# tdavchev/DESIRE

Hardware: AMD Instinct MI355X
Metric: agent-trajectory-samples/sec (K=20, T_pred=40) (higher is better)
Workload: dtype f32; 1 GPU; BASELINE configs[1]: SDD-like synthetic windows, 32 agent slots/window, K=20, T_obs=8/T_pred=40, H=128, L=128, fp32, posterior CVAE, IOC 1 refinement, social grid 4x4, scene grid 64x64x32; 512 windows/step/GPU; windows_per_gpu=512, rows_per_gpu=327680, parallelism=scene-sharded x1

## Files before the change

### desire_amd/_build.py

```python
from __future__ import annotations

import hashlib
import os
import shutil
import subprocess
from concurrent.futures import ThreadPoolExecutor

HERE = os.path.dirname(os.path.abspath(__file__))
CSRC = os.path.join(HERE, "csrc")
LIB = os.path.join(HERE, "libdesire_hip.so")
SOURCES = ["api.hip", "api_pack.hip", "api_forward.hip", "api_peer.hip", "api_ops.hip", "kernels_gemm.hip", "kernels_conv.hip", "kernels_rnn.hip", "kernels_aux.hip", "kernels_rank.hip", "kernels_kde.hip", "kernels_select.hip", "kernels_joint.hip", "kernels_worlds.hip", "kernels_plan.hip", "kernels_modes.hip", "kernels_scene_modes.hip", "kernels_occ.hip", "kernels_recon.hip", "kernels_compact.hip", "kernels_bwd.hip", "kernels_bwd_x3.hip", "kernels_bwd_cl.hip", "kernels_bf16.hip", "kernels_bf16_cl.hip", "kernels_x3.hip", "kernels_x6.hip", "kernels_x6r2.hip", "kernels_scene.hip", "kernels_rng.hip", "kernels_rollout.hip", "train.hip", "backward.hip"]
FLAGS = ["--offload-arch=gfx950", "-O3", "-std=c++17", "-fPIC", "-Wno-unused-value", "-Wno-pass-failed"]
FLAGS += os.environ.get("DESIRE_HIPCC_FLAGS", "").split()
_SINK = ["-mllvm", "-sink-insts-to-avoid-spills"]
FILE_FLAGS = {f: list(_SINK) for f in ("kernels_bf16_cl.hip", "kernels_x3.hip")}
_extra = os.environ.get("DESIRE_FILE_FLAGS", "")
for _item in filter(None, _extra.split(";")):
    _f, _, _v = _item.partition("=")
    FILE_FLAGS[_f] = [x for x in _v.split(",") if x]


def _sha(paths, extra: str = "") -> str:
    h = hashlib.sha256(extra.encode())
    for p in paths:
        h.update(os.path.basename(p).encode())
        with open(p, "rb") as fh:
            h.update(fh.read())
    return h.hexdigest()


def _headers():
    return sorted(os.path.join(CSRC, f) for f in os.listdir(CSRC) if f.endswith(".h")) + [os.path.join(HERE, "..", "include", "desire_hip.h")]


def source_hash() -> str:
    srcs = sorted(os.path.join(CSRC, f) for f in os.listdir(CSRC) if f.endswith(".hip"))
    return _sha(srcs + _headers(), " ".join(FLAGS) + repr(sorted(FILE_FLAGS.items())))[:16]


def _read(path: str) -> str:
    try:
        with open(path) as fh:
            return fh.read().strip()
    except OSError:
        return ""


def build_lib(force: bool = False, verbose: bool = False) -> str:
    want = source_hash()
    objdir = os.path.join(HERE, "build")
    lib_stamp = os.path.join(objdir, "lib.stamp")
    if not force and os.path.exists(LIB) and _read(lib_stamp) == want:
        return LIB
    hipcc = shutil.which("hipcc") or "/opt/rocm/bin/hipcc"
    if not os.path.exists(hipcc):
        raise RuntimeError("hipcc not found: cannot build libdesire_hip.so")
    os.makedirs(objdir, exist_ok=True)
    hdrs = _headers()

    def cc(src: str) -> str:
        obj = os.path.join(objdir, src.replace(".hip", ".o"))
        flags = list(FLAGS) + FILE_FLAGS.get(src, [])
        if src == "api.hip":
            flags.append('-DDESIRE_SRC_HASH="%s"' % want)
        key = _sha([os.path.join(CSRC, src)] + hdrs, " ".join(flags))
        if not force and os.path.exists(obj) and _read(obj + ".stamp") == key:
            return obj
        cmd = [hipcc, *flags, "-c", os.path.join(CSRC, src), "-o", obj]
        r = subprocess.run(cmd, capture_output=True, text=True)
        if r.returncode != 0:
            raise RuntimeError("hipcc failed on %s:\n%s" % (src, r.stderr[-4000:]))
        if verbose and r.stderr:
            print(r.stderr)
        with open(obj + ".stamp", "w") as fh:
            fh.write(key)
        return obj

    with ThreadPoolExecutor(len(SOURCES)) as ex:
        objs = list(ex.map(cc, SOURCES))
    r = subprocess.run([hipcc, "--offload-arch=gfx950", "-shared", "-fPIC", "-o", LIB, *objs],
                       capture_output=True, text=True)
    if r.returncode != 0:
        raise RuntimeError("link failed:\n" + r.stderr[-4000:])
    with open(lib_stamp, "w") as fh:
        fh.write(want)
    return LIB


if __name__ == "__main__":
    print(build_lib(force=True, verbose=True))
```

### desire_amd/_lib.py

```python
from __future__ import annotations

import ctypes as C
import os
from typing import Dict, List, Tuple

import numpy as np

from .spec import Dims

LIB_PATH = os.environ.get("DESIRE_HIP_LIB") or os.path.join(os.path.dirname(os.path.abspath(__file__)), "libdesire_hip.so")

EXPORTS = [
    "desire_last_error", "desire_version", "desire_dims_size", "desire_build_hash", "desire_create", "desire_destroy", "desire_set_weight",
    "desire_finalize_weights", "desire_set_scene_grids", "desire_set_scene_images", "desire_encode", "desire_sample",
    "desire_ioc_refine", "desire_forward", "desire_read_buffer", "desire_neighbor_bins",
    "desire_scene_cells", "desire_set_profiling", "desire_get_profile", "desire_scene_cnn", "desire_losses",
    "desire_temporal_conv", "desire_feature_pooling", "desire_build_windows", "desire_gaussian_sample", "desire_ade_fde",
    "desire_set_training", "desire_backward", "desire_get_grad", "desire_grad_buffer",
    "desire_train_loss", "desire_adam_step", "desire_get_weight", "desire_clip_grads",
    "desire_device_buffer", "desire_ioc_step", "desire_ioc_finish", "desire_get_bin_table",
    "desire_graph_begin", "desire_graph_end", "desire_graph_launch", "desire_rollout", "desire_build_windows_la", "desire_adam_state",
    "desire_set_option", "desire_train_loss_async", "desire_set_head_loss",
    "desire_peer_export", "desire_peer_open", "desire_ioc_peer_pass", "desire_peer_close", "desire_peer_region", "desire_peer_open_ptr", "desire_peer_status",
    "desire_rank_samples", "desire_ranked_errors", "desire_kde_nll", "desire_select_diverse", "desire_joint_metrics",
    "desire_set_rng", "desire_set_rng_origin", "desire_rng_state", "desire_rng_fill", "desire_rollout_samples",
    "desire_set_recon_loss", "desire_recon_weights", "desire_occupancy", "desire_plan_risk", "desire_fit_modes",
    "desire_select_worlds", "desire_fit_scene_modes",
]
OCC_AT, OCC_UNTIL = 0, 1
OCC_MODES = {"at": OCC_AT, "until": OCC_UNTIL}
RNG_BITS, RNG_NORMAL, RNG_LATENT, RNG_ROLLOUT = 0, 1, 2, 3
DIST_FINAL, DIST_MEAN, DIST_MAX = 0, 1, 2
WORLD_ALL, WORLD_MEAN = 0, 1
RECON_MEAN, RECON_MIN, RECON_SOFTMIN = 0, 1, 2
RECON_MODES = {"mean": RECON_MEAN, "min": RECON_MIN, "softmin": RECON_SOFTMIN}
MODES_MAX, MODES_MAX_ITERS = 16, 32
KDE_LOG_FLOOR = -20.0


class DesireDims(C.Structure):
    _fields_ = [(n, C.c_int32) for n in
                ("n_scenes", "mno", "K", "T_obs", "T_pred", "H", "L", "S", "C", "Gh", "Gw", "n_grids",
                 "grid_size", "E_v", "iters", "posterior")] + \
               [(n, C.c_float) for n in ("nb_w", "nb_h", "sx", "sy")] + [(n, C.c_int32) for n in ("bin_mode", "bn_mode", "bf16", "ref_compat", "n_dec", "ioc_form", "ioc_split", "train_fp32_mask", "flags")]

    @classmethod
    def from_dims(cls, d: Dims) -> "DesireDims":
        return cls(d.n_scenes, d.mno, d.K, d.T_obs, d.T_pred, d.H, d.L, d.S, d.C, d.Gh, d.Gw, d.n_grids,
                   d.grid_size, d.E_v, d.iters, d.posterior, d.nb_w, d.nb_h, d.sx, d.sy, int(getattr(d, "bin_mode", 0)),
                   int(getattr(d, "bn_mode", 0)), int(getattr(d, "bf16", 0)), int(getattr(d, "ref_compat", 0)), int(getattr(d, "n_dec", 0)),
                   int(getattr(d, "ioc_form", 0)), int(getattr(d, "ioc_split", 0)), int(getattr(d, "train_fp32_mask", 0)), int(getattr(d, "flags", 0)))


class DesireError(RuntimeError):
    pass


_lib = None


def load() -> C.CDLL:
    global _lib
    if _lib is not None:
        return _lib
    try:
        import torch
    except ImportError:
        pass
    if not os.path.exists(LIB_PATH):
        raise DesireError(
            "libdesire_hip.so not found at %s -- run `python -c 'import __graft_entry__ as g; g.build()'`; "
            "desire_amd has no CPU fallback" % LIB_PATH)
    lib = C.CDLL(LIB_PATH)
    vp, i32, f32p = C.c_void_p, C.c_int32, C.c_void_p
    lib.desire_last_error.restype = C.c_char_p
    lib.desire_build_hash.restype = C.c_char_p
    lib.desire_create.argtypes = [C.POINTER(DesireDims), C.POINTER(vp)]
    lib.desire_destroy.argtypes = [vp]
    lib.desire_set_option.argtypes = [vp, C.c_char_p, i32]
    lib.desire_set_weight.argtypes = [vp, C.c_char_p, C.POINTER(C.c_float), C.c_size_t]
    lib.desire_finalize_weights.argtypes = [vp]
    lib.desire_set_scene_grids.argtypes = [vp, f32p, C.POINTER(C.c_int32)]
    lib.desire_set_scene_images.argtypes = [vp, f32p, i32, i32, C.POINTER(C.c_int32)]
    lib.desire_encode.argtypes = [vp, f32p, f32p, vp]
    lib.desire_sample.argtypes = [vp, f32p, f32p, vp]
    lib.desire_ioc_refine.argtypes = [vp, f32p, f32p, vp]
    lib.desire_forward.argtypes = [vp, f32p, f32p, f32p, f32p, f32p, vp]
    lib.desire_read_buffer.argtypes = [vp, C.c_char_p, C.POINTER(C.c_float), C.c_size_t, vp]
    lib.desire_neighbor_bins.argtypes = [vp, f32p, vp, vp, i32, vp]
    lib.desire_scene_cells.argtypes = [vp, f32p, vp, i32, vp]
    lib.desire_scene_cnn.argtypes = [vp, f32p, i32, i32, f32p, vp]
    lib.desire_losses.argtypes = [vp, f32p, f32p, f32p, f32p, f32p, vp]
    lib.desire_temporal_conv.argtypes = [vp, f32p, f32p, vp]
    lib.desire_feature_pooling.argtypes = [vp, f32p, f32p, f32p, vp]
    lib.desire_build_windows.argtypes = [vp, f32p, i32, i32, C.POINTER(C.c_int32), i32, f32p, f32p, vp]
    lib.desire_build_windows_la.argtypes = [vp, f32p, i32, i32, C.POINTER(C.c_int32), i32, i32, f32p, f32p, vp]
    lib.desire_gaussian_sample.argtypes = [vp, f32p, f32p, f32p, i32, vp]
    lib.desire_ade_fde.argtypes = [vp, f32p, f32p, f32p, vp]
    lib.desire_rank_samples.argtypes = [vp, f32p, f32p, i32, vp, f32p, f32p, vp]
    lib.desire_ranked_errors.argtypes = [vp, f32p, f32p, vp, i32, C.POINTER(C.c_int32), i32, C.c_float, C.c_float, f32p, vp]
    lib.desire_kde_nll.argtypes = [vp, f32p, f32p, f32p, C.POINTER(C.c_int32), i32, C.c_float, C.c_float, C.c_float, f32p, f32p, vp]
    lib.desire_select_diverse.argtypes = [vp, f32p, vp, f32p, i32, i32, C.c_float, C.c_float, C.c_float, i32, vp, vp, f32p, f32p, f32p, vp]
    lib.desire_joint_metrics.argtypes = [vp, f32p, f32p, vp, f32p, C.POINTER(C.c_int32), i32, i32, C.c_float, C.c_float, C.c_float, vp, vp, f32p, f32p,
                                         vp, f32p, vp]
    lib.desire_select_worlds.argtypes = [vp, f32p, vp, f32p, i32, i32, i32, C.c_float, C.c_float, C.c_float, vp, vp, f32p, vp, vp]
    lib.desire_occupancy.argtypes = [vp, f32p, f32p, vp, f32p, C.POINTER(C.c_int32), i32, i32, i32, i32, vp, vp, f32p, f32p, f32p, f32p, f32p, vp]
    lib.desire_plan_risk.argtypes = [vp, f32p, f32p, vp, f32p, f32p, vp, i32, C.POINTER(C.c_int32), i32, C.c_float, C.c_float, C.c_float, vp, f32p, f32p, f32p, vp]
    lib.desire_fit_modes.argtypes = [vp, f32p, vp, f32p, f32p, i32, i32, i32, C.c_float, C.c_float, C.c_float, C.POINTER(C.c_int32), i32, C.c_float,
                                     vp, vp, f32p, f32p, f32p, vp, f32p, f32p, vp]
    lib.desire_fit_scene_modes.argtypes = [vp, f32p, vp, vp, f32p, f32p, i32, i32, i32, C.c_float, C.c_float, C.c_float, C.POINTER(C.c_int32), i32,
                                           C.c_float, vp, vp, f32p, f32p, f32p, vp, f32p, f32p, vp]
    lib.desire_rollout.argtypes = [vp, f32p, f32p, i32, f32p, vp]
    lib.desire_rollout_samples.argtypes = [vp, f32p, f32p, f32p, vp]
    lib.desire_set_training.argtypes = [vp, C.c_int]
    lib.desire_backward.argtypes = [vp, f32p, f32p, f32p, vp]
    lib.desire_get_grad.argtypes = [vp, C.c_char_p, C.POINTER(C.c_float), C.c_size_t, vp]
    lib.desire_grad_buffer.argtypes = [vp, C.POINTER(C.c_void_p), C.POINTER(C.c_size_t)]
    lib.desire_train_loss.argtypes = [vp, f32p, C.POINTER(C.c_float), vp]
    lib.desire_train_loss_async.argtypes = [vp, f32p, f32p, vp]
    lib.desire_set_head_loss.argtypes = [vp, C.c_float]
    lib.desire_set_recon_loss.argtypes = [vp, i32, C.c_float]
    lib.desire_recon_weights.argtypes = [vp, f32p, f32p, i32, C.c_float, f32p, f32p, vp, f32p, vp]
    lib.desire_peer_export.argtypes = [vp, C.c_char_p, C.POINTER(C.c_size_t)]
    lib.desire_peer_open.argtypes = [vp, i32, i32, i32, C.c_char_p]
    lib.desire_ioc_peer_pass.argtypes = [vp, f32p, f32p, vp]
    lib.desire_peer_close.argtypes = [vp]
    lib.desire_peer_status.argtypes = [vp, C.POINTER(C.c_int32)]
    lib.desire_peer_region.argtypes = [vp, C.POINTER(C.c_void_p), C.POINTER(C.c_size_t)]
    lib.desire_peer_open_ptr.argtypes = [vp, i32, i32, i32, vp]
    lib.desire_adam_step.argtypes = [vp, C.c_float, C.c_float, C.c_float, C.c_float, vp]
    lib.desire_adam_state.argtypes = [vp, C.POINTER(C.c_int32), C.c_int]
    lib.desire_get_weight.argtypes = [vp, C.c_char_p, C.POINTER(C.c_float), C.c_size_t, vp]
    lib.desire_clip_grads.argtypes = [vp, C.c_float, C.POINTER(C.c_float), vp]
    lib.desire_get_bin_table.argtypes = [vp, C.POINTER(C.c_float)]
    lib.desire_graph_begin.argtypes = [vp, vp]
    lib.desire_graph_end.argtypes = [vp, vp, C.POINTER(C.c_int32)]
    lib.desire_graph_launch.argtypes = [vp, i32, vp]
    lib.desire_device_buffer.argtypes = [vp, C.c_char_p, C.POINTER(C.c_void_p), C.POINTER(C.c_size_t)]
    lib.desire_ioc_step.argtypes = [vp, i32, i32, i32, f32p, f32p, vp, f32p, f32p, f32p, vp]
    lib.desire_ioc_finish.argtypes = [vp, f32p, f32p, f32p, f32p, vp]
    lib.desire_set_rng.argtypes = [vp, C.c_uint64, C.c_uint32, vp]
    lib.desire_set_rng_origin.argtypes = [vp, C.c_uint32, C.c_uint32]
    lib.desire_rng_state.argtypes = [vp, C.POINTER(C.c_uint32), vp]
    lib.desire_rng_fill.argtypes = [vp, C.c_uint64, C.c_uint32, C.c_uint64, i32, vp, C.c_size_t, vp]
    lib.desire_set_profiling.argtypes = [vp, C.c_int]
    lib.desire_get_profile.argtypes = [vp, C.POINTER(C.c_float), C.POINTER(C.c_char_p), C.POINTER(C.c_int32)]
    for n in EXPORTS:
        if n not in ("desire_last_error", "desire_build_hash"):
            getattr(lib, n).restype = C.c_int
    if lib.desire_dims_size() != C.sizeof(DesireDims):
        raise DesireError("libdesire_hip.so was built with sizeof(desire_dims) = %d, this binding has %d: rebuild (python -c 'import "
                          "__graft_entry__ as g; g.build()')" % (lib.desire_dims_size(), C.sizeof(DesireDims)))
    _lib = lib
    return lib


def _chk(rc: int) -> None:
    if rc != 0:
        raise DesireError("libdesire_hip error %d: %s" % (rc, load().desire_last_error().decode()))


def _horizons(horizons, optional: bool = False):
    if optional and horizons is None:
        return np.zeros(0, np.int32), None
    hz = np.ascontiguousarray(horizons, dtype=np.int32).reshape(-1)
    return hz, hz.ctypes.data_as(C.POINTER(C.c_int32))


class Handle:

    def __init__(self, dims: Dims):
        dims.validate()
        self.dims = dims
        self.lib = load()
        self._h = C.c_void_p()
        cd = DesireDims.from_dims(dims)
        _chk(self.lib.desire_create(C.byref(cd), C.byref(self._h)))

    def close(self) -> None:
        if getattr(self, "_h", None) is not None and self._h:
            self.lib.desire_destroy(self._h)
            self._h = C.c_void_p()

    def __del__(self):
        try:
            self.close()
        except Exception:
            pass

    def set_option(self, name: str, value: int) -> None:
        _chk(self.lib.desire_set_option(self._h, name.encode(), int(value)))
        if hasattr(self.dims, name):
            self.dims = self.dims.replace(**{name: int(value)})

    def set_weights(self, weights: Dict[str, np.ndarray]) -> None:
        for name, arr in weights.items():
            a = np.ascontiguousarray(arr, dtype=np.float32)
            _chk(self.lib.desire_set_weight(self._h, name.encode(), a.ctypes.data_as(C.POINTER(C.c_float)), a.size))
        _chk(self.lib.desire_finalize_weights(self._h))

    def set_scene_grids(self, dev_grids_ptr: int, grid_of_scene) -> None:
        g = np.ascontiguousarray(grid_of_scene, dtype=np.int32)
        if g.size != self.dims.n_scenes:
            raise DesireError("grid_of_scene must have n_scenes entries")
        _chk(self.lib.desire_set_scene_grids(self._h, dev_grids_ptr, g.ctypes.data_as(C.POINTER(C.c_int32))))

    def set_scene_images(self, dev_images_ptr: int, Hi: int, Wi: int, grid_of_scene) -> None:
        g = np.ascontiguousarray(grid_of_scene, dtype=np.int32)
        if g.size != self.dims.n_scenes:
            raise DesireError("grid_of_scene must have n_scenes entries")
        _chk(self.lib.desire_set_scene_images(self._h, dev_images_ptr, int(Hi), int(Wi), g.ctypes.data_as(C.POINTER(C.c_int32))))

    def encode(self, past_ptr: int, fut_ptr: int, stream: int = 0) -> None:
        _chk(self.lib.desire_encode(self._h, past_ptr, fut_ptr or None, stream or None))

    def sample(self, eps_ptr: int, yhat_ptr: int, stream: int = 0) -> None:
        _chk(self.lib.desire_sample(self._h, eps_ptr, yhat_ptr, stream or None))

    def set_rng(self, seed: int, draw: int = 0, stream: int = 0) -> None:
        _chk(self.lib.desire_set_rng(self._h, int(seed) & (2 ** 64 - 1), int(draw) & 0xFFFFFFFF, stream or None))

    def set_rng_origin(self, scene_base: int = 0, slot_base: int = 0) -> None:
        _chk(self.lib.desire_set_rng_origin(self._h, int(scene_base) & 0xFFFFFFFF, int(slot_base) & 0xFFFFFFFF))

    def rng_state(self, stream: int = 0) -> Tuple[int, int]:
        out = (C.c_uint32 * 2)()
        _chk(self.lib.desire_rng_state(self._h, out, stream or None))
# ... 191 lines not shown
    def clip_grads(self, max_norm: float, want_norm: bool = False, stream: int = 0):
        out = C.c_float(0.0)
        _chk(self.lib.desire_clip_grads(self._h, C.c_float(max_norm), C.byref(out) if want_norm else None, stream or None))
        return float(out.value) if want_norm else None

    def train_loss(self, fut_ptr: int, stream: int = 0) -> Dict[str, float]:
        out = (C.c_float * 5)()
        _chk(self.lib.desire_train_loss(self._h, fut_ptr, out, stream or None))
        return self.loss_terms(self.read_buffer("loss_out", (8,), stream))

    def peer_export(self) -> bytes:
        buf = C.create_string_buffer(64)
        n = C.c_size_t(0)
        _chk(self.lib.desire_peer_export(self._h, buf, C.byref(n)))
        return bytes(buf.raw)

    def peer_open(self, rank: int, nranks: int, peer: int, handle: bytes = None) -> None:
        _chk(self.lib.desire_peer_open(self._h, rank, nranks, peer, None if peer == rank else bytes(handle)))

    def peer_region(self) -> int:
        p, n = C.c_void_p(), C.c_size_t(0)
        _chk(self.lib.desire_peer_region(self._h, C.byref(p), C.byref(n)))
        return int(p.value)

    def peer_open_ptr(self, rank: int, nranks: int, peer: int, region_ptr: int = 0) -> None:
        _chk(self.lib.desire_peer_open_ptr(self._h, rank, nranks, peer, region_ptr or None))

    def ioc_peer_pass(self, y_ptr: int, score_ptr: int, stream: int = 0) -> None:
        _chk(self.lib.desire_ioc_peer_pass(self._h, y_ptr, score_ptr, stream or None))

    def peer_timed_out(self) -> bool:
        v = C.c_int32(0)
        _chk(self.lib.desire_peer_status(self._h, C.byref(v)))
        return bool(v.value)

    def peer_close(self) -> None:
        _chk(self.lib.desire_peer_close(self._h))

    def set_head_loss(self, weight: float) -> None:
        _chk(self.lib.desire_set_head_loss(self._h, C.c_float(float(weight))))

    def set_recon_loss(self, mode: int, tau: float = 0.0) -> None:
        _chk(self.lib.desire_set_recon_loss(self._h, int(mode), C.c_float(float(tau))))

    def recon_weights(self, fut_ptr: int, yhat_ptr: int, mode: int, tau: float = 0.0, e_ptr: int = 0, w_ptr: int = 0, winner_ptr: int = 0,
                      recon_ptr: int = 0, stream: int = 0) -> None:
        _chk(self.lib.desire_recon_weights(self._h, fut_ptr or None, yhat_ptr or None, int(mode), C.c_float(float(tau)), e_ptr or None, w_ptr or None,
                                           winner_ptr or None, recon_ptr or None, stream or None))

    def train_loss_async(self, fut_ptr: int, out8_ptr: int, stream: int = 0) -> None:
        _chk(self.lib.desire_train_loss_async(self._h, fut_ptr, out8_ptr, stream or None))

    @staticmethod
    def loss_terms(v8) -> Dict[str, float]:
        v8 = [float(x) for x in list(v8)[:8]]
        r = dict(zip(("recon", "kld", "ce", "reg", "n_present", "nll_head", "grad_norm", "n_head"), v8))
        r["loss"] = r["recon"] + r["kld"] + r["ce"] + r["reg"] + r["nll_head"]
        return r

    def adam_step(self, lr: float = 0.005, beta1: float = 0.9, beta2: float = 0.999, eps: float = 1e-8, stream: int = 0) -> None:
        _chk(self.lib.desire_adam_step(self._h, C.c_float(lr), C.c_float(beta1), C.c_float(beta2), C.c_float(eps), stream or None))

    def opt_state(self) -> Dict[str, np.ndarray]:
        t = C.c_int32(0)
        _chk(self.lib.desire_adam_state(self._h, C.byref(t), 0))
        return {"m": self.device_tensor("Mflat").cpu().numpy(), "v": self.device_tensor("Vflat").cpu().numpy(),
                "t": np.array([t.value], np.int64)}

    def set_opt_state(self, st: Dict[str, np.ndarray]) -> None:
        import torch
        m, v = self.device_tensor("Mflat"), self.device_tensor("Vflat")
        if st["m"].size != m.numel() or st["v"].size != v.numel():
            raise DesireError("optimiser state of %d values does not fit this model (%d)" % (st["m"].size, m.numel()))
        m.copy_(torch.as_tensor(np.ascontiguousarray(st["m"], np.float32), device=m.device))
        v.copy_(torch.as_tensor(np.ascontiguousarray(st["v"], np.float32), device=v.device))
        t = C.c_int32(int(np.asarray(st["t"]).reshape(-1)[0]))
        _chk(self.lib.desire_adam_state(self._h, C.byref(t), 1))

    def get_weight(self, name: str, shape: Tuple[int, ...], stream: int = 0) -> np.ndarray:
        out = np.empty(shape, np.float32)
        _chk(self.lib.desire_get_weight(self._h, name.encode(), out.ctypes.data_as(C.POINTER(C.c_float)), out.size, stream or None))
        return out

    def set_profiling(self, on: bool) -> None:
        _chk(self.lib.desire_set_profiling(self._h, int(on)))

    def get_profile(self) -> List[Tuple[str, float]]:
        n0 = C.c_int32(1 << 30)
        _chk(self.lib.desire_get_profile(self._h, None, None, C.byref(n0)))
        cap = max(int(n0.value), 1)
        ms = (C.c_float * cap)()
        names = (C.c_char_p * cap)()
        n = C.c_int32(cap)
        _chk(self.lib.desire_get_profile(self._h, ms, names, C.byref(n)))
        return [(names[i].decode(), float(ms[i])) for i in range(n.value)]
```

### desire_amd/csrc/api.hip

```cpp
#include "ctx.h"

#include <cmath>
#include <cstdio>
#include <cstdlib>
#include <cstring>

static thread_local std::string g_err;
int desire_fail(int code, const std::string& msg) { g_err = msg; return code; }

extern "C" const char* desire_last_error(void) { return g_err.c_str(); }
extern "C" int desire_version(void) { return 5; }
extern "C" int desire_dims_size(void) { return (int)sizeof(desire_dims); }
#ifndef DESIRE_SRC_HASH
#define DESIRE_SRC_HASH "unstamped"
#endif
extern "C" const char* desire_build_hash(void) { return DESIRE_SRC_HASH; }

int desire_upload(desire_ctx* h, const std::string& name, const std::vector<float>& v) {
    const size_t bytes = v.size() * sizeof(float);
    const DevBuf* b = h->dev.find(name.c_str());
    if (!b || b->bytes != bytes) {
        h->dev.release(name.c_str());
        if (h->dev.ensure(name.c_str(), bytes)) return -1;
    }
    return hipMemcpy(h->dev.get(name.c_str()), v.data(), bytes, hipMemcpyHostToDevice) == hipSuccess ? 0 : -1;
}

static void embed_walk(const Embed& em, const std::function<void(size_t, size_t)>& f) {
    size_t cl = 0, cp = 0;
    for (auto& c : em.cols.seg) { cl += c.first; cp += c.second; }
    size_t rl = 0, rp = 0;
    for (auto& r : em.rows.seg) {
        for (int i = 0; i < r.first; ++i) {
            size_t ol = 0, op = 0;
            for (auto& c : em.cols.seg) {
                for (int j = 0; j < c.first; ++j) f((rl + i) * cl + ol + j, (rp + i) * cp + op + j);
                ol += c.first; op += c.second;
            }
        }
        rl += r.first; rp += r.second;
    }
}
std::vector<float> desire_embed(const desire_ctx* h, const std::string& name, const float* user) {
    auto it = h->emb.find(name);
    const size_t np = h->want.at(name);
    if (it == h->emb.end()) return std::vector<float>(user, user + np);
    std::vector<float> out(np, 0.f);
    embed_walk(it->second, [&](size_t il, size_t ip) { out[ip] = user[il]; });
    return out;
}
void desire_extract(const desire_ctx* h, const std::string& name, const float* phys, float* user) {
    auto it = h->emb.find(name);
    if (it == h->emb.end()) { std::memcpy(user, phys, h->want.at(name) * sizeof(float)); return; }
    embed_walk(it->second, [&](size_t il, size_t ip) { user[il] = phys[ip]; });
}

namespace {

void embeddings(desire_ctx* h) {
    const desire_dims& d = h->d;
    const std::pair<int, int> Hs{h->Hl, d.H};
    auto fix = [](int n) { return std::pair<int, int>{n, n}; };
    auto& e = h->emb;
    auto gru = [&](const std::string& p, std::vector<std::pair<int, int>> in) {
        in.push_back(Hs);
        e[p + "/gates/kernel"] = Embed{{in}, {{Hs, Hs}}};
        e[p + "/gates/bias"] = Embed{{{fix(1)}}, {{Hs, Hs}}};
        e[p + "/candidate/kernel"] = Embed{{in}, {{Hs}}};
        e[p + "/candidate/bias"] = Embed{{{fix(1)}}, {{Hs}}};
    };
    gru("enc_x", {fix(2)}); gru("enc_y", {fix(2)}); gru("dec", {Hs}); gru("ioc", {fix(d.E_v + d.C), Hs});
    e["fc_c/w"] = Embed{{{Hs, Hs}}, {{fix(h->V)}}};
    e["mask_fc/w"] = Embed{{{fix(h->V)}}, {{Hs}}};
    e["mask_fc/b"] = Embed{{{fix(1)}}, {{Hs}}};
    e["head/w"] = Embed{{{Hs}}, {{fix(2)}}};
    e["ioc/social_fc/w"] = Embed{{std::vector<std::pair<int, int>>(h->B, Hs)}, {{Hs}}};
    e["ioc/social_fc/b"] = Embed{{{fix(1)}}, {{Hs}}};
    e["ioc/score/w"] = Embed{{{Hs}}, {{fix(1)}}};
    e["ioc/reg/w"] = Embed{{{Hs}}, {{fix(2 * d.T_pred)}}};
    e["gauss_head/w"] = Embed{{{Hs}}, {{fix(5)}}};
}

int check_options(const desire_dims& d) {
    switch (d.ioc_form) {
        case DESIRE_IOC_AUTO: case DESIRE_IOC_TILE64: case DESIRE_IOC_CLUSTER: case DESIRE_IOC_CLUSTER_BINS: case DESIRE_IOC_COMPACT:
        case DESIRE_IOC_TRAIN_DENSE: case DESIRE_IOC_X6_TILE32: case DESIRE_IOC_X6_TILE64: break;
        default: return fail(DESIRE_ERR_ARG, "ioc_form must be one of DESIRE_IOC_* (include/desire_hip.h)");
    }
    if (d.ioc_split < 0 || d.ioc_split > 4) return fail(DESIRE_ERR_ARG, "ioc_split must be 0 (auto), 1 (never split: batch-size invariant results) or 2..4 (cap)");
    if (d.train_fp32_mask < 0 || d.train_fp32_mask > 15) return fail(DESIRE_ERR_ARG, "train_fp32_mask is a mask of bits 1, 2, 4, 8");
    if (d.flags & ~(DESIRE_FLAG_NO_FUSE34 | DESIRE_FLAG_TRAIN_FWD_3P | DESIRE_FLAG_COMPACT_ROWS | DESIRE_FLAG_COMPACT_IOC)) return fail(DESIRE_ERR_ARG, "unknown bit in flags (DESIRE_FLAG_*)");
    if ((d.flags & DESIRE_FLAG_COMPACT_IOC) && d.ref_compat) return fail(DESIRE_ERR_ARG, "DESIRE_FLAG_COMPACT_IOC: ref_compat has no IOC stage");
    if ((d.flags & DESIRE_FLAG_COMPACT_ROWS) && (d.bn_mode == 2 || d.ref_compat))
        return fail(DESIRE_ERR_ARG, "DESIRE_FLAG_COMPACT_ROWS: not with bn_mode = 2 (whole-batch statistics depend on the padding rows) or ref_compat");
    return 0;
}

int check_dims(const desire_dims& d) {
    if (d.S != 32) return fail(DESIRE_ERR_ARG, "S must be 32 (rnn_size=512): CVAE stack shapes, model/model.py:465-468");
    if (d.mno < 1 || d.mno > 256 || (d.mno <= 32 ? (32 % d.mno) : (d.mno % 32)))
        return fail(DESIRE_ERR_ARG, "mno must divide 32 or be a multiple of 32 up to 256 (above 128: inference, step-wise IOC)");
    if (d.mno > 128 && d.bf16 == 1) return fail(DESIRE_ERR_ARG, "more than 128 agents per scene run the fp32 step-wise IOC (bf16 = 0, 2 or 3)");
    if (d.H != 16 && d.H != 32 && d.H != 64 && d.H != 128 && d.H != 256)
        return fail(DESIRE_ERR_ARG, "H must be 16, 32 (run zero-padded on the 64-wide tile), 64, 128 or 256");

    if (d.L % 8 || d.L < 8) return fail(DESIRE_ERR_ARG, "L must be a positive multiple of 8");
    if (d.C != 32 || d.E_v != 16) return fail(DESIRE_ERR_ARG, "C=32 and E_v=16 are the instantiated IOC widths in this round");
    if (d.n_scenes < 1 || d.K < 1 || d.T_obs < 1 || d.T_pred < 1 || d.n_grids < 1 || d.iters < 1 || d.Gh < 1 || d.Gw < 1)
        return fail(DESIRE_ERR_ARG, "sizes must be >= 1");
    if (d.grid_size < 1 || d.grid_size > 6) return fail(DESIRE_ERR_ARG, "grid_size must be 1..6 (6 x 6 = the paper's 36 bins)");
    if (d.grid_size > 4 && d.H == 256) return fail(DESIRE_ERR_ARG, "grid_size 5..6 needs H <= 128 (LDS budget of the IOC tile)");
    if (d.bf16 < 0 || d.bf16 > 3)
        return fail(DESIRE_ERR_ARG, "bf16 must be 0 (fp32 operands), 1 (bf16 operands), 2 (split-bf16 operands: hi + lo, three products) or 3 (three "
                                    "bf16 pieces, six products: fp32-class accuracy)");
    if (d.bn_mode < 0 || d.bn_mode > 2) return fail(DESIRE_ERR_ARG, "bn_mode must be 0 (frozen statistics), 1 (per-object statistics) or 2 (whole-batch statistics)");
    if (d.bn_mode && d.bf16 == 1) return fail(DESIRE_ERR_ARG, "batch statistics (bn_mode 1 / 2) run on fp32 operands (bf16 = 0 or 2)");
    if (d.bin_mode != 0 && d.bin_mode != 1) return fail(DESIRE_ERR_ARG, "bin_mode must be 0 (rectangular) or 1 (log-polar)");
    if (d.bin_mode == 1 && (d.grid_size < 3 || !(d.nb_h > 0.f) || !(d.nb_w > d.nb_h)))
        return fail(DESIRE_ERR_ARG, "log-polar bins: grid_size >= 3 and 0 < nb_h (inner radius) < nb_w (outer radius)");
    if (!(d.nb_w > 0.f) || !(d.nb_h > 0.f)) return fail(DESIRE_ERR_ARG, "nb_w/nb_h must be > 0");
    if (d.ref_compat != 0 && d.ref_compat != 1) return fail(DESIRE_ERR_ARG, "ref_compat must be 0 or 1");
    if (int rc = check_options(d)) return rc;
    if (d.ref_compat) {
        if (d.K != 1 || !d.posterior || d.bn_mode != 1 || d.bf16 || d.n_dec < 1 || d.H != 2 * d.T_obs || d.T_pred != d.T_obs)
            return fail(DESIRE_ERR_ARG, "ref_compat (the reference graph as written, model/model.py:116-311) needs K = 1 (one eps per object, "
                                        ":262-263), posterior = 1, bn_mode = 1, bf16 = 0, H == 2*T_obs (:286-289), T_pred == T_obs and n_dec >= 1 (:280 runs 7)");
    } else if (d.n_dec != 0) return fail(DESIRE_ERR_ARG, "n_dec belongs to ref_compat (0 otherwise)");
    return 0;
}

}

extern "C" int desire_set_option(desire_handle* h, const char* name, int32_t value) {
    if (!h || !name) return fail(DESIRE_ERR_ARG, "null argument");
    desire_dims d = h->d;
    const std::string nm(name);
    if (nm == "ioc_form") d.ioc_form = value;
    else if (nm == "ioc_split") d.ioc_split = value;
    else if (nm == "train_fp32_mask") d.train_fp32_mask = value;
    else if (nm == "flags") d.flags = value;
    else if (nm == "compact_host_counts") {
        h->cp_host_counts = value != 0;
        h->cp_pending = false; h->cp_enc = false;
        return DESIRE_OK;
    }
    else if (nm == "scene_grad") {
        if (value != 0 && value != 1) return fail(DESIRE_ERR_ARG, "scene_grad must be 0 or 1");
        h->scene_grad = value != 0;
        return scene_grad_on(h) && h->training ? scene_grad_setup(h) : DESIRE_OK;
    }
    else if (nm == "compact_min_rows") {
        if (value < 0) return fail(DESIRE_ERR_ARG, "compact_min_rows must be >= 0");
        h->ci_min_rows = value;
        return DESIRE_OK;
    }
    else if (nm == "scene_modes_chunk") {
        if (value < 0) return fail(DESIRE_ERR_ARG, "scene_modes_chunk must be >= 0");
        h->scene_modes_chunk = value;
        return DESIRE_OK;
    }
    else return fail(DESIRE_ERR_ARG, "unknown option: " + nm + " (ioc_form, ioc_split, train_fp32_mask, flags, compact_min_rows, compact_host_counts, scene_grad, scene_modes_chunk)");
    if (int rc = check_options(d)) return rc;
    if (((d.flags ^ h->d.flags) & (DESIRE_FLAG_COMPACT_ROWS | DESIRE_FLAG_COMPACT_IOC)) ||
        ((d.flags & DESIRE_FLAG_COMPACT_IOC) && (d.ioc_form != h->d.ioc_form || d.train_fp32_mask != h->d.train_fp32_mask)))
        h->cp_pending = h->cp_enc = false;
    h->d = d;
    return DESIRE_OK;
}

extern "C" int desire_create(const desire_dims* dims, desire_handle** out) {
    if (!dims || !out) return fail(DESIRE_ERR_ARG, "null argument");
    if (int rc = check_dims(*dims)) return rc;
    int ndev = 0;
    if (hipGetDeviceCount(&ndev) != hipSuccess || ndev < 1)
        return fail(DESIRE_ERR_NODEV, "no HIP device: libdesire_hip has no CPU path");
    int dev = 0;
    HIPCHK(hipGetDevice(&dev));
    hipDeviceProp_t prop;
    HIPCHK(hipGetDeviceProperties(&prop, dev));
    if (std::strncmp(prop.gcnArchName, "gfx950", 6) != 0)
        return fail(DESIRE_ERR_NODEV, std::string("device is ") + prop.gcnArchName + ", kernels are built for gfx950 only");
    desire_ctx* h = new desire_ctx();
    h->d = *dims;
    h->Hl = dims->H;
    if (dims->H < 64) h->d.H = 64;
    h->A = dims->n_scenes * dims->mno;
    h->R = h->A * dims->K;
    h->V = dims->S * dims->S;
    h->B = dims->grid_size * dims->grid_size;
    h->E = dims->E_v + dims->C + h->d.H;
    pack::weight_shapes(h->d, h->d.H, h->V, h->B, h->want);
    pack::weight_shapes(h->d, h->Hl, h->V, h->B, h->want_user);
    if (h->Hl != h->d.H) embeddings(h);
    const desire_dims& d = h->d;
    const size_t A = h->A, R = h->R, f = sizeof(float);
    const WsItem list[] = {
        {"HxHy", A * 2 * d.H * f}, {"p_last", A * 2 * f}, {"valid", A}, {"lmask", A}, {"nfut", A * f}, {"vae_in", A * h->V * f},
        {"c1", A * 8192 * f}, {"c2", A * 4096 * f}, {"c3", A * 2048 * f}, {"params", A * 2 * d.L * f},
        {"z", R * d.L * f}, {"d1", R * 2048 * f}, {"d2", R * 4096 * f}, {"d3", R * 8192 * f},
        {"xhat", R * 1024 * f}, {"xz", R * d.H * f}, {"Y0", R * (size_t)(d.n_dec > d.T_pred ? d.n_dec : d.T_pred) * 2 * f},
        {"dec_states", d.ref_compat ? R * (size_t)d.n_dec * d.H * f : 0},
        {"bn_part", d.bn_mode == 2 ? (size_t)512 * 128 * f : 0}, {"bn_stat", d.bn_mode == 2 ? (size_t)2 * 128 * f : 0},
        {"grid_of_scene", (size_t)d.n_scenes * sizeof(int32_t)},
        {"bw_starts", (size_t)d.n_scenes * sizeof(int32_t)}, {"bw_err", sizeof(int32_t)},
        {"rank_tab", d.ref_compat ? 0 : R * 16 * f}, {"rank_cnt", d.ref_compat ? 0 : A * 8 * sizeof(int32_t)},
        {"kde_w", d.ref_compat ? 0 : R * f}, {"kde_st", d.ref_compat ? 0 : A * 2 * f},
        {"joint_js", d.ref_compat ? 0 : (size_t)d.n_scenes * d.K * f}, {"joint_je", d.ref_compat ? 0 : (size_t)d.n_scenes * d.K * 16 * f},
    };
    if (int rc = ws_ensure(h, list)) { desire_destroy(h); return rc; }
    for (const WsItem& w : list) (void)hipMemset(W(h, w.n), 0, w.bytes);
    h->bw_starts = Wt<int32_t>(h, "bw_starts"); h->bw_err = Wt<int32_t>(h, "bw_err");
    if (d.bin_mode == 1) {
        std::vector<float> tab(20, 0.f);
        const int G = d.grid_size;
        for (int k = 0; k < G; ++k) {
            const float t = (float)((double)d.nb_h * std::pow((double)d.nb_w / (double)d.nb_h, (double)(k + 1) / G));
            tab[k] = t * t;
            tab[8 + 2 * k] = (float)std::cos(2.0 * M_PI * k / G);
            tab[9 + 2 * k] = (float)std::sin(2.0 * M_PI * k / G);
        }
        h->bin_tab_host = tab;
        if (int rc = ws_ensure(h, {{"bin_tab", 20 * f}})) { desire_destroy(h); return rc; }
        if (hipMemcpy(W(h, "bin_tab"), tab.data(), 20 * f, hipMemcpyHostToDevice) != hipSuccess) { desire_destroy(h); return fail(DESIRE_ERR_HIP, "bin table upload failed"); }
    }
    *out = h;
    return DESIRE_OK;
}

extern "C" int desire_get_bin_table(desire_handle* h, float* host_out20) {
    if (!h || !host_out20) return fail(DESIRE_ERR_ARG, "null argument");
    if (h->d.bin_mode != 1) return fail(DESIRE_ERR_STATE, "the rectangular grid has no table (dims.bin_mode = 0)");
    std::memcpy(host_out20, h->bin_tab_host.data(), 20 * sizeof(float));
    return DESIRE_OK;
}

extern "C" int desire_peer_close(desire_handle* h);
extern "C" int desire_destroy(desire_handle* h) {
    if (!h) return DESIRE_OK;
    if (h->host_err) { (void)hipHostFree(h->host_err); h->host_err = nullptr; }
    if (h->cp_host) { (void)hipHostFree(h->cp_host); h->cp_host = nullptr; }
    if (h->cp_ev) { (void)hipEventDestroy(h->cp_ev); h->cp_ev = nullptr; }
    (void)desire_peer_close(h);
    h->dev.release_all();
    h->ws.release_all();
    for (auto& p : h->prof) { (void)hipEventDestroy(p.e0); (void)hipEventDestroy(p.e1); }
    for (void* g : h->graphs) if (g) (void)hipGraphExecDestroy(static_cast<hipGraphExec_t>(g));
    delete h;
    return DESIRE_OK;
}

extern "C" int desire_set_weight(desire_handle* h, const char* name, const float* host_data, size_t n) {
    if (!h || !name || !host_data) return fail(DESIRE_ERR_ARG, "null argument");
    auto it = h->want_user.find(name);
    if (it == h->want_user.end()) return fail(DESIRE_ERR_ARG, std::string("unknown weight: ") + name);
    if (it->second != n)
        return fail(DESIRE_ERR_ARG, std::string("weight ") + name + ": expected " + std::to_string(it->second) +
                                        " values, got " + std::to_string(n));
    h->host_w[name] = desire_embed(h, name, host_data);
    h->finalized = false;
    h->img_stale = true;
    h->training = false;
    return DESIRE_OK;
}

extern "C" int desire_finalize_weights(desire_handle* h) {
    if (!h) return fail(DESIRE_ERR_ARG, "null handle");
    for (auto& kv : h->want)
        if (!h->host_w.count(kv.first)) return fail(DESIRE_ERR_STATE, "weight not set: " + kv.first);
    if (int rc = desire_pack_all(h)) return rc;
    h->finalized = true;
    h->img_stale = true;
    return DESIRE_OK;
}

extern "C" int desire_set_scene_grids(desire_handle* h, const float* dev_grids, const int32_t* host_grid_of_scene) {
    if (!h || !dev_grids || !host_grid_of_scene) return fail(DESIRE_ERR_ARG, "null argument");
    for (int i = 0; i < h->d.n_scenes; ++i)
        if (host_grid_of_scene[i] < 0 || host_grid_of_scene[i] >= h->d.n_grids)
            return fail(DESIRE_ERR_ARG, "grid_of_scene entry out of range");
    HIPCHK(hipMemcpy(W(h, "grid_of_scene"), host_grid_of_scene, h->d.n_scenes * sizeof(int32_t), hipMemcpyHostToDevice));
    h->grids = dev_grids;
    h->grids_set = true;
    h->img_set = false; h->img = nullptr;
    return DESIRE_OK;
}

extern "C" int desire_set_scene_images(desire_handle* h, const float* dev_images, int32_t Hi, int32_t Wi, const int32_t* host_grid_of_scene) {
    if (!h || !dev_images || !host_grid_of_scene) return fail(DESIRE_ERR_ARG, "null argument");
    const desire_dims& d = h->d;
    if (Hi != 4 * d.Gh || Wi != 4 * d.Gw) return fail(DESIRE_ERR_ARG, "scene image must be [n_grids, 4*Gh, 4*Gw, 3]");
// ... 7 lines not shown
}

int desire_ready(desire_handle* h) {
    if (!h) return fail(DESIRE_ERR_ARG, "null handle");
    if (!h->finalized) return fail(DESIRE_ERR_STATE, "weights not finalized (desire_finalize_weights)");
    return 0;
}

extern "C" int desire_read_buffer(desire_handle* h, const char* name, float* host_out, size_t n, void* stream) {
    if (!h || !name || !host_out) return fail(DESIRE_ERR_ARG, "null argument");
    hipStream_t s = static_cast<hipStream_t>(stream);
    HIPCHK(hipStreamSynchronize(s));
    const desire_dims& d = h->d;
    const size_t A = h->A, R = h->R, f = sizeof(float);
    const std::string nm(name);
    auto strided = [&](const float* src, size_t cols, size_t pitch_cols, size_t rows) -> int {
        if (n != rows * cols) return fail(DESIRE_ERR_ARG, nm + ": expected " + std::to_string(rows * cols) + " values");
        HIPCHK(hipMemcpy2D(host_out, cols * f, src, pitch_cols * f, cols * f, rows, hipMemcpyDeviceToHost));
        return 0;
    };
    if (nm == "Hx") return strided(W(h, "HxHy"), h->Hl, 2 * d.H, A);
    if (nm == "Hy") return strided(W(h, "HxHy") + d.H, h->Hl, 2 * d.H, A);
    if (nm == "xz") return strided(W(h, "xz"), h->Hl, d.H, R);
    if (nm == "z_mean") return strided(W(h, "params"), d.L, 2 * d.L, A);
    if (nm == "z_log_sigma_sq") return strided(W(h, "params") + d.L, d.L, 2 * d.L, A);
    struct P { const char* n; size_t cnt; };
    const P plain[] = {{"vae_in", A * h->V}, {"c1", A * 8192}, {"c2", A * 4096}, {"c3", A * 2048}, {"z", R * d.L},
                       {"d1", R * 2048}, {"d2", R * 4096}, {"d3", R * 8192}, {"xhat", R * 1024},
                       {"Y0", R * d.T_pred * 2}, {"p_last", A * 2}};
    for (const P& p : plain)
        if (nm == p.n) {
            if (n != p.cnt) return fail(DESIRE_ERR_ARG, nm + ": expected " + std::to_string(p.cnt) + " values");
            HIPCHK(hipMemcpy(host_out, W(h, p.n), p.cnt * f, hipMemcpyDeviceToHost));
            return DESIRE_OK;
        }
    {
        if (const DevBuf* b = h->ws.find(name)) {
            if (n * f > b->bytes) return fail(DESIRE_ERR_ARG, nm + ": holds " + std::to_string(b->bytes / f) + " values");
            HIPCHK(hipMemcpy(host_out, b->p, n * f, hipMemcpyDeviceToHost));
            return DESIRE_OK;
        }
    }
    return fail(DESIRE_ERR_ARG, "unknown buffer: " + nm);
}

extern "C" int desire_graph_begin(desire_handle* h, void* stream) {
    if (int rc = desire_ready(h)) return rc;
    if (!stream) return fail(DESIRE_ERR_ARG, "graph capture needs an explicit (non-default) stream");
    if (h->profiling) return fail(DESIRE_ERR_STATE, "switch profiling off before capturing (event records are not part of the graph)");
    HIPCHK(hipStreamBeginCapture(static_cast<hipStream_t>(stream), hipStreamCaptureModeThreadLocal));
    return DESIRE_OK;
}

extern "C" int desire_graph_end(desire_handle* h, void* stream, int32_t* graph_id) {
    if (!h || !stream || !graph_id) return fail(DESIRE_ERR_ARG, "null argument");
    hipGraph_t g = nullptr;
    HIPCHK(hipStreamEndCapture(static_cast<hipStream_t>(stream), &g));
    hipGraphExec_t ex = nullptr;
    const hipError_t e = hipGraphInstantiate(&ex, g, nullptr, nullptr, 0);
    (void)hipGraphDestroy(g);
    if (e != hipSuccess) return fail(DESIRE_ERR_HIP, std::string("hipGraphInstantiate: ") + hipGetErrorString(e));
    h->graphs.push_back(ex);
    *graph_id = (int32_t)h->graphs.size() - 1;
    return DESIRE_OK;
}

extern "C" int desire_graph_launch(desire_handle* h, int32_t graph_id, void* stream) {
    if (!h) return fail(DESIRE_ERR_ARG, "null handle");
    if (graph_id < 0 || graph_id >= (int32_t)h->graphs.size() || !h->graphs[graph_id]) return fail(DESIRE_ERR_ARG, "unknown graph id");
    HIPCHK(hipGraphLaunch(static_cast<hipGraphExec_t>(h->graphs[graph_id]), static_cast<hipStream_t>(stream)));
    return DESIRE_OK;
}

extern "C" int desire_device_buffer(desire_handle* h, const char* name, void** dev_ptr, size_t* bytes) {
    if (!h || !name || !dev_ptr || !bytes) return fail(DESIRE_ERR_ARG, "null argument");
    if (!std::strcmp(name, "scene_grid_grad") && !(scene_grad_on(h) && h->training))
        return fail(DESIRE_ERR_STATE, "scene_grid_grad needs training mode and desire_set_option(h, \"scene_grad\", 1)");
    const DevBuf* b = h->ws.find(name);
    if (!b) return fail(DESIRE_ERR_ARG, std::string("unknown buffer: ") + name);
    *dev_ptr = b->p; *bytes = b->bytes;
    return DESIRE_OK;
}

extern "C" int desire_set_profiling(desire_handle* h, int enable) {
    if (!h) return fail(DESIRE_ERR_ARG, "null handle");
    h->profiling = enable != 0;
    return DESIRE_OK;
}

extern "C" int desire_get_profile(desire_handle* h, float* host_ms, const char** host_names, int32_t* count) {
    if (!h || !count) return fail(DESIRE_ERR_ARG, "null argument");
    const int cap = *count;
    int n = 0;
    for (auto& p : h->prof) {
        if (n >= cap) break;
        HIPCHK(hipEventSynchronize(p.e1));
        float ms = 0.f;
        HIPCHK(hipEventElapsedTime(&ms, p.e0, p.e1));
        if (host_ms) host_ms[n] = ms;
        if (host_names) host_names[n] = p.name.c_str();
        ++n;
    }
    *count = n;
    if (!host_ms && !host_names) return DESIRE_OK;
    h->prof_name_store.clear();
    for (auto& p : h->prof) h->prof_name_store.push_back(p.name);
    if (host_names) for (int i = 0; i < n; ++i) host_names[i] = h->prof_name_store[i].c_str();
    for (auto& p : h->prof) { (void)hipEventDestroy(p.e0); (void)hipEventDestroy(p.e1); }
    h->prof.clear();
    return DESIRE_OK;
}
```

### desire_amd/csrc/api_forward.hip

```cpp
#include "ctx.h"

#include <cmath>
#include <cstdio>
#include <cstdlib>
#include <cstring>

bool compact_rows(const desire_ctx* h) { return (h->d.flags & DESIRE_FLAG_COMPACT_ROWS) != 0; }
bool compact_ioc(const desire_ctx* h) { return (h->d.flags & DESIRE_FLAG_COMPACT_IOC) && ioc_plan(h).fwd != IocFwd::STEPWISE; }
ClassLayout class_layout(const desire_ctx* h, bool pad, const int* counts) {
    const desire_dims& d = h->d;
    ClassLayout L;
    int cand[6], nc = 0;
    for (int m : {8, 10, 16, 32, 64, 96}) if (m < d.mno && (m != 10 || pad)) cand[nc++] = m;
    for (int i = nc > 3 ? nc - 3 : 0; i < nc; ++i) L.m[L.n++] = cand[i];
    L.m[L.n++] = d.mno;
    for (int i = L.n; i < 4; ++i) L.m[i] = d.mno;
    for (int c = 0; c < L.n; ++c) {
        IocView& v = L.c[c];
        v.cls = c; v.mno = L.m[c]; v.n_scenes = counts ? counts[c] : d.n_scenes;
        v.gpt = (v.mno <= 32 && 32 % v.mno) ? 32 / v.mno : 0; v.ngrp = v.n_scenes * d.K;
        v.R = v.gpt ? (long)((v.ngrp + v.gpt - 1) / v.gpt) * 32 : (long)v.ngrp * v.mno;
        v.agent_off = L.agents; v.row_off = L.rows; v.win_off = L.wins;
        L.agents += (size_t)v.n_scenes * v.mno; L.rows += (size_t)v.R; L.wins += (size_t)v.n_scenes;
    }
// ... 289 lines not shown
    a.xz = W(h, "xz"); a.Hx = HxS; a.ldhx = 2 * H; a.p_last = plS;
    a.R = R; a.K = d.K; a.mno = mno; a.H = H; a.T = d.T_pred;
    a.Wxg = D4(h, "dec/Wxg"); a.Wxc = D4(h, "dec/Wxc"); gen_op2(h, GenStage::DECODER, plan.decoder, a.Whg, a.Whc);
    a.b_g = D(h, "dec/gb"); a.b_c = D(h, "dec/cb"); a.w_head = D(h, "head/w"); a.b_head = D(h, "head/b");
    a.Y = Yout; a.hdump = nullptr; a.dyn = DynCount{dynP, 1, hintS};
    if (d.ref_compat) { a.T = d.n_dec; a.hdump = W(h, "dec_states"); }
    if (h->training) { a.hdump = W(h, "dec_sv_h"); a.sv_r = W(h, "dec_sv_r"); a.sv_u = W(h, "dec_sv_u"); a.sv_c = W(h, "dec_sv_c"); }
    { Timer t(h, s, "decoder");
      switch (plan.decoder) {
          case GenForm::BF16: launch_decoder_bf16(a, s); break;
          case GenForm::X6: launch_decoder_x6(a, s, plan.np); break;
          case GenForm::FP32: launch_decoder(a, s);
      } }
    if (d.ref_compat)
        launch_copy_cols(dev_Yhat, W(h, "dec_states"), (size_t)R * d.n_dec, h->Hl, H, s);
    else if (compact) {
        Timer t(h, s, "compact_scatter");
        const size_t RT2 = (size_t)h->R * d.T_pred * 2;
        launch_fill_f32(W(h, "Y0"), RT2, 0.f, s); launch_fill_f32(dev_Yhat, RT2, 0.f, s);
        launch_scatter_rows(Yout, W(h, "Y0"), dev_Yhat, Wt<const int32_t>(h, "cp_amap"), mno, d.K, d.mno, d.T_pred * 2, s, dynP);
    } else
        launch_copy_f32(dev_Yhat, W(h, "Y0"), (size_t)R * d.T_pred * 2, s);
    HIPCHK(hipGetLastError());
    return DESIRE_OK;
}

int ioc_cluster_exchange(desire_ctx* h, size_t n_groups, bool reset_err, hipStream_t s) {
    if (int rc = ws_ensure(h, {{"hex", (size_t)2 * h->R * h->d.H * sizeof(float)}, {"grp_cnt", ((size_t)h->R / 32 + 1) * sizeof(int)}, {"ioc_err", sizeof(int)}})) return rc;
    HIPCHK(hipMemsetAsync(W(h, "grp_cnt"), 0, n_groups * sizeof(int), s));
    if (reset_err) HIPCHK(hipMemsetAsync(W(h, "ioc_err"), 0, sizeof(int), s));
    return DESIRE_OK;
}
int ioc_cluster_check(desire_ctx* h, hipStream_t s, const char* what) {
    int err = 0;
    HIPCHK(hipMemcpyAsync(&err, W(h, "ioc_err"), sizeof(int), hipMemcpyDeviceToHost, s));
    HIPCHK(hipStreamSynchronize(s));
    return err ? fail(DESIRE_ERR_HIP, std::string(what) + " hand-off timed out (workgroups of a group were not co-resident)") : DESIRE_OK;
}
#ifdef DESIRE_IOC_TIMING
void ioc_timing_report(const long long* dbg, const char* const* names, int n, hipStream_t s) {
    long long host[16];
    (void)hipStreamSynchronize(s); (void)hipMemcpy(host, dbg, n * sizeof(long long), hipMemcpyDeviceToHost);
    long long tot = 0; for (int k = 0; k < n; ++k) tot += host[k];
    for (int k = 0; k < n; ++k) fprintf(stderr, "[ioc timing] %-45s %12lld cyc  %5.1f%%\n", names[k], host[k], 100.0 * host[k] / (double)tot);
}
#endif

static int ioc_core(desire_handle* h, const IocView& v, hipStream_t s) {
    const desire_dims& d = h->d;
    if (h->training && d.bf16 == 1) return fail(DESIRE_ERR_STATE, "bf16 operands are inference-only");
    IocArgs a{};
    a.Y = v.Y; a.score = v.score; a.Hx = v.Hx; a.ldhx = 2 * d.H; a.p_last = v.p_last; a.valid = v.valid;
    a.R = (int)v.R; a.K = d.K; a.mno = v.mno; a.H = d.H; a.T = d.T_pred; a.iters = d.iters;
    a.C = d.C; a.Gh = d.Gh; a.Gw = d.Gw; a.E_v = d.E_v; a.G = d.grid_size; a.nb_w = d.nb_w; a.nb_h = d.nb_h;
    a.grids = h->grids; a.grid_of_scene = v.gos; a.bin_tab = d.bin_mode == 1 ? W(h, "bin_tab") : nullptr;
    a.w_vel = D(h, "ioc/vel_w"); a.b_vel = D(h, "ioc/vel_b");
    a.Wsoc = D4(h, "ioc/Wsoc"); a.b_soc = D(h, "ioc/soc_b"); a.Wsoc_c = D4(h, "ioc/Wsoc_c");
    a.Wg = D4(h, "ioc/Wg"); a.Wc = D4(h, "ioc/Wc"); a.b_g = D(h, "ioc/gb"); a.b_c = D(h, "ioc/cb");
    a.w_score = D(h, "ioc/score_w"); a.b_score = D(h, "ioc/score_b");
    a.Wreg = D4(h, "ioc/Wreg"); a.b_reg = D(h, "ioc/reg_b"); a.NTreg = (2 * d.T_pred + 31) / 32;
    a.variant = d.ioc_form; a.gpt = v.gpt; a.ngrp = v.ngrp; a.dyn = DynCount{v.dynN, 1, 0};
    const IocPlan p = ioc_plan(d, h->training, v.mno, v.gpt, v.R, [&](int n) { return ioc_bin_split_capacity(a, n); });
    if (!p.fp32_weights()) { a.Wsoc = D4(h, "ioc/Wsoc16"); a.Wg = D4(h, "ioc/Wg16"); a.Wc = D4(h, "ioc/Wc16"); a.Wreg = D4(h, "ioc/Wreg16"); }
    if (p.cluster()) {
        if (int rc = ioc_cluster_exchange(h, (size_t)v.R / v.mno, true, s)) return rc;
        a.hex = W(h, "hex"); a.grp_cnt = Wt<int>(h, "grp_cnt"); a.err = Wt<int>(h, "ioc_err");
    }
    if (p.nspl > 1) {
        const size_t tiles = ((size_t)v.R + 31) / 32, tiles_max = ((size_t)h->R + 31) / 32;
        if (int rc = ws_ensure(h, {{"hex_s", tiles_max * 2 * 4 * 32 * d.H * sizeof(float)}, {"cnt_s", tiles_max * sizeof(int)}})) return rc;
        if (!h->host_err) {
            if (hipHostMalloc(reinterpret_cast<void**>(&h->host_err), sizeof(int), hipHostMallocMapped) != hipSuccess || !h->host_err)
                { h->host_err = nullptr; return fail(DESIRE_ERR_HIP, "hipHostMalloc failed for the bin-split error word"); }
            *h->host_err = 0;
        }
        if (*static_cast<volatile int*>(h->host_err)) {
            *h->host_err = 0;
            return fail(DESIRE_ERR_HIP, "bin-split IOC hand-off timed out in an earlier call (workgroups of a tile were not co-resident)");
        }
        launch_fill_f32(W(h, "cnt_s"), tiles, 0.f, s);
        a.hex = W(h, "hex_s"); a.grp_cnt = Wt<int>(h, "cnt_s"); a.err = h->host_err;
        a.nspl = p.nspl;
    }
#ifdef DESIRE_IOC_TIMING
    if (int rc = ws_ensure(h, {{"dbg", 10 * sizeof(long long)}})) return rc;
    a.dbg = Wt<long long>(h, "dbg");
#endif
    const int passes = h->training ? d.iters : 1;
    if (h->training) a.iters = 1;
    for (int it = 0; it < passes; ++it) {
        if (h->training) {
            const size_t po = ioc_save_off(h, it, v);
            launch_copy_f32(W(h, "ioc_Yin") + po * 2, v.Y, (size_t)v.R * d.T_pred * 2, s);
            a.sv_x = W(h, "ioc_sv_x") + po * h->E; a.sv_r = W(h, "ioc_sv_r") + po * d.H; a.sv_u = W(h, "ioc_sv_u") + po * d.H;
            a.sv_c = W(h, "ioc_sv_c") + po * d.H; a.sv_h = W(h, "ioc_sv_h") + po * d.H;
            if (p.cluster() && it > 0) { if (int rc = ioc_cluster_exchange(h, (size_t)v.R / v.mno, false, s)) return rc; }
        }
        Timer t(h, s, "ioc");
        switch (p.fwd) {
            case IocFwd::FP32: case IocFwd::FP32_WIDE: launch_ioc(a, p.fwd == IocFwd::FP32_WIDE, s); break;
            case IocFwd::FP32_CLUSTER: launch_ioc_cluster(a, s); break;
            case IocFwd::BF16: case IocFwd::BF16_WIDE: launch_ioc_bf16(a, p.fwd == IocFwd::BF16_WIDE, s); break;
            case IocFwd::BF16_CLUSTER: if (launch_ioc_bf16_cluster(a, s)) return fail(DESIRE_ERR_HIP, "bf16 cluster IOC: no resident grid for this shape"); break;
            case IocFwd::X3: launch_ioc_x3(a, s); break;
            case IocFwd::X3R2: launch_ioc_x3r2(a, s); break;
            case IocFwd::X6: launch_ioc_x6(a, s); break;
            case IocFwd::X6R2: launch_ioc_x6r2(a, s); break;
            case IocFwd::STEPWISE: return fail(DESIRE_ERR_STATE, "the step-wise IOC has no view form");
        }
    }
#ifdef DESIRE_IOC_TIMING
    const char* n32[9] = {"P0 pos+clear", "P1 ev/es/masks", "build0+bar", "build(b+1)", "mma bin", "bin barrier", "P3 e_r+bar", "P4 gates(2 mma)+ep+2bar", "P5 cand+ep+2bar"};
    const char* n16[9] = {"loop top", "P1 ev/es/masks", "barrier 1", "P2 pooling chain + e_r", "barrier 2", "P4 gates + r*h", "barrier 3", "P5 cand + publish", "barrier 4"};
    const char* nx3[10] = {"step top (bar 4 wait)", "P1 ev/es/masks", "barrier 1", "P2 pooling chain", "exchange + e_r", "barrier 2", "P4 gates + r*h", "barrier 3", "P5 cand + publish", "barrier 4"};
    const char* ncl[10] = {"step top: positions + clear + bar", "P1 ev/es/masks", "wait for the peers", "copy peers' Ht + bar", "P2 pooling chains",
                           "exchange + e_r", "barrier 2", "P4 gates + r*h + cand frags", "bar 3 + P5 cand + publish stores", "drain + arrive + bar"};
    const bool split = !p.fp32_weights() && d.bf16 != 1, cl16 = p.fwd == IocFwd::BF16_CLUSTER;
    ioc_timing_report(a.dbg, split ? nx3 : cl16 ? ncl : d.bf16 == 1 ? n16 : n32, split || cl16 ? 10 : 9, s);
#endif
    HIPCHK(hipGetLastError());
    return p.cluster() ? ioc_cluster_check(h, s, "IOC cluster") : DESIRE_OK;
}

extern "C" int desire_ioc_refine(desire_handle* h, float* dev_Yhat, float* dev_score, void* stream) {
    if (int rc = desire_ready(h)) return rc;
    if (!dev_Yhat || !dev_score) return fail(DESIRE_ERR_ARG, "null argument");
    if (h->d.ref_compat) return fail(DESIRE_ERR_STATE, "ref_compat: the reference graph has no ranking/refinement module (model/model.py:312-313)");
    if (!h->grids_set) return fail(DESIRE_ERR_STATE, "scene grids not set (desire_set_scene_grids)");
    if (h->img_set && (h->training || h->img_stale)) {
        if (int rc = scene_images_run(h, static_cast<hipStream_t>(stream))) return rc;
    }
    const desire_dims& d = h->d;
    hipStream_t s = static_cast<hipStream_t>(stream);
    if (ioc_plan(h).fwd == IocFwd::STEPWISE) {
        if (h->training) return fail(DESIRE_ERR_STATE, "training supports up to 128 agents per scene");
        const size_t RH = (size_t)h->R * d.H;
        if (int rc = ws_ensure(h, {{"stw_h", 2 * RH * sizeof(float)}, {"stw_sc", (size_t)h->R * sizeof(float)}})) return rc;
        float* hb[2] = {W(h, "stw_h"), W(h, "stw_h") + RH};
        const int NTs = d.H / 32, KXs = d.E_v + d.C + 2 * d.H;
        for (int it = 0; it < d.iters; ++it) {
            launch_hx_rows(hb[1], W(h, "HxHy"), 2 * d.H, d.n_scenes, d.K, d.mno, d.H, s);
            Timer tm(h, s, "ioc");
            for (int t = 0; t < d.T_pred; ++t) {
                IocStepArgs q = ioc_step_args(h, t);
                q.rank = 0; q.nranks = 1;
                q.Yall = dev_Yhat; q.plast_all = W(h, "p_last"); q.valid_all = Wt<const uint8_t>(h, "valid"); q.Hall = hb[(t + 1) & 1];
                q.st_h = hb[(t + 1) & 1]; q.st_h_out = hb[t & 1]; q.st_score = W(h, "stw_sc");
                if (d.bf16 == 2 || d.bf16 == 3) {
                    q.np = d.bf16 == 3 ? 3 : 2;
                    q.Wsoc = D4(h, "ioc/Wsoc16l"); q.Wg = D4(h, "ioc/Wg16"); q.Wc = D4(h, "ioc/Wc16");
                    q.plo_soc = (size_t)d.grid_size * d.grid_size * NTs * (d.H / 16) * 64; q.plo_g = (size_t)2 * NTs * (KXs / 16) * 64; q.plo_c = (size_t)NTs * (KXs / 16) * 64;
                }
                launch_ioc_step(q, s);
            }
            if (int rc = desire_ioc_finish(h, hb[(d.T_pred - 1) & 1], W(h, "stw_sc"), dev_Yhat, dev_score, stream)) return rc;
        }
        HIPCHK(hipGetLastError());
        return DESIRE_OK;
    }
    if (compact_ioc(h)) {
        if (int rc = compact_wait(h, s)) return rc;
        const bool pad = ioc_plan(h).padded, dyn = compact_dyn(h);
        int cnt[4] = {0, 0, 0, 0};
        for (int c = 0, n = class_layout(h, pad, nullptr).n; c < n; ++c) {
            cnt[c] = dyn ? d.n_scenes : static_cast<volatile const int32_t*>(h->cp_host + 4)[c];
            if (cnt[c] < 0 || cnt[c] > d.n_scenes) return fail(DESIRE_ERR_HIP, "slot-class scan returned a count out of range");
        }
        const ClassLayout L = class_layout(h, pad, cnt);
        const int T2 = d.T_pred * 2;
        launch_fill_f32(dev_score, (size_t)h->R, 0.f, s);
        for (int c = 0; c < 4; ++c) h->ci_cnt[c] = c < L.n ? L.c[c].n_scenes : 0;
        for (int c = 0; c < L.n; ++c) {
            if (L.c[c].n_scenes == 0) continue;
            IocView v = ioc_view(h, &L.c[c]);
            if (dyn) v.dynN = Wt<const int32_t>(h, "cp_count") + 4 + c;
            {
                Timer t(h, s, "ioc_repack");
                launch_cls_gather_agents(W(h, "HxHy"), 2 * d.H, W(h, "p_last"), Wt<const int32_t>(h, "grid_of_scene"), v.cmap, v.win, v.n_scenes, v.mno,
                                         v.Hx, v.p_last, v.valid, v.gos, s, v.dynN);
                launch_cls_rows(dev_Yhat, v.Y, v.cmap, v.n_scenes, v.mno, d.K, d.mno, T2, 0, s, v.gpt, v.dynN);
            }
// ... 30 lines not shown
```

### desire_amd/csrc/ctx.h

```cpp
#pragma once
#include "../../include/desire_hip.h"
#include "gen_plan.h"
#include "ioc_plan.h"
#include "kernels.h"
#include "pack.h"
#include "workspace.h"

#include <hip/hip_runtime.h>

#include <cstring>
#include <functional>
#include <map>
#include <string>
#include <vector>

int desire_fail(int code, const std::string& msg);
#define fail desire_fail
#define HIPCHK(x)                                                                                   \
    do {                                                                                            \
        hipError_t e_ = (x);                                                                        \
        if (e_ != hipSuccess)                                                                       \
            return fail(DESIRE_ERR_HIP, std::string(#x) + ": " + hipGetErrorString(e_));            \
    } while (0)

inline int dev_malloc(void** p, size_t bytes) { return hipMalloc(p, bytes) == hipSuccess ? 0 : -1; }
inline void dev_free(void* p) { (void)hipFree(p); }

struct Prof { std::string name; hipEvent_t e0, e1; };

struct WSlot { size_t off; size_t n; };

struct EmbedAxis { std::vector<std::pair<int, int>> seg; };
struct Embed { EmbedAxis rows, cols; };

struct desire_ctx {
    desire_dims d;
    int Hl = 0;
    int A, R, V, B, E;
    std::map<std::string, size_t> want_user;
    std::map<std::string, Embed> emb;
    std::map<std::string, std::vector<float>> host_w;
    std::map<std::string, size_t> want;
    Workspace dev{dev_malloc, dev_free};
    Workspace ws{dev_malloc, dev_free};
    bool finalized = false;
    std::vector<void*> graphs;
    std::vector<float> bin_tab_host;
    const float* grids = nullptr;
    bool grids_set = false;
    bool profiling = false;
    void* peer_region = nullptr; size_t peer_bytes = 0; void* peer_base[8] = {nullptr, nullptr, nullptr, nullptr, nullptr, nullptr, nullptr, nullptr};
    bool peer_mapped[8] = {false, false, false, false, false, false, false, false}; int peer_rank = -1, peer_nranks = 0; bool peer_ready = false;
    int* peer_err = nullptr;
    float head_loss_w = 0.f;
    int recon_mode = 0; float recon_tau = 0.f;
    int* host_err = nullptr;
    int32_t* cp_host = nullptr; hipEvent_t cp_ev = nullptr; bool cp_pending = false; int cp_P = -1;
    int ci_cnt[4] = {0, 0, 0, 0}; bool ci_last = false; int ci_min_rows = 8192;
    bool cp_enc = false;
    bool cp_host_counts = false;
    bool cp_last = false;
    int scene_modes_chunk = 0;
    int32_t* bw_starts = nullptr; int32_t* bw_err = nullptr;
    uint32_t* rng_state = nullptr; uint32_t rng_scene_base = 0, rng_slot_base = 0;
    std::vector<Prof> prof;
    std::vector<std::string> prof_name_store;
    bool training = false;
    std::map<std::string, WSlot> slots;
    size_t n_params = 0;
    const float* last_eps = nullptr;
    int adam_t = 0;
    int n_seg = 0;
    int n_seg16 = 0;
    bool scene_grad = false;
    const float* img = nullptr; bool img_set = false;
    bool img_stale = true;
};

struct Timer {
    desire_ctx* h; hipStream_t s; bool on; size_t idx = 0;
    Timer(desire_ctx* h_, hipStream_t s_, const char* name) : h(h_), s(s_), on(h_->profiling) {
        if (!on) return;
        Prof p; p.name = name;
        (void)hipEventCreate(&p.e0); (void)hipEventCreate(&p.e1);
        (void)hipEventRecord(p.e0, s);
        idx = h->prof.size();
        h->prof.push_back(p);
    }
    ~Timer() { if (on) (void)hipEventRecord(h->prof[idx].e1, s); }
};

inline GenPlan gen_plan(const desire_ctx* h) { return gen_plan(h->d, h->training, h->V); }

inline const float* D(desire_ctx* h, const char* name) { return h->dev.get(name); }
inline const float4* D4(desire_ctx* h, const char* name) { return h->dev.get<const float4>(name); }
inline float* W(desire_ctx* h, const char* name) { return h->ws.get(name); }
template <class T> T* Wt(desire_ctx* h, const char* name) { return h->ws.get<T>(name); }
template <size_t N> int ws_ensure(desire_ctx* h, const WsItem (&list)[N]) {
    std::string failed;
    return h->ws.ensure_all(list, N, &failed) ? fail(DESIRE_ERR_HIP, "hipMalloc failed for " + failed) : 0;
}

std::vector<float> desire_embed(const desire_ctx* h, const std::string& name, const float* user);
void desire_extract(const desire_ctx* h, const std::string& name, const float* phys, float* user);
int desire_upload(desire_ctx* h, const std::string& name, const std::vector<float>& v);
int desire_ready(desire_handle* h);
bool compact_rows(const desire_ctx* h);
bool compact_ioc(const desire_ctx* h);
bool compact_dyn(const desire_ctx* h);
int compact_setup(desire_ctx* h);
inline IocPlan ioc_plan(const desire_ctx* h) { return ioc_plan(h->d, h->training, h->d.mno, 0, h->R); }
struct IocView {
    int cls = -1, mno = 0, n_scenes = 0, gpt = 0, ngrp = 0;
    long R = 0;
    size_t agent_off = 0, row_off = 0, win_off = 0;
    float* Hx = nullptr; float* p_last = nullptr; uint8_t* valid = nullptr; int32_t* gos = nullptr;
    const int32_t* cmap = nullptr; const int32_t* win = nullptr;
    float* Y = nullptr; float* score = nullptr; const int32_t* dynN = nullptr;
};
struct ClassLayout { int n = 0; int m[4] = {0, 0, 0, 0}; IocView c[4]; size_t agents = 0, rows = 0, wins = 0; };
ClassLayout class_layout(const desire_ctx* h, bool pad, const int* counts);
IocView ioc_view(desire_ctx* h, const IocView* cls = nullptr);
inline size_t ioc_save_rows(const desire_ctx* h) { return (size_t)h->R + 128; }
inline size_t ioc_save_off(const desire_ctx* h, int pass, const IocView& v) { return ((size_t)pass * ioc_save_rows(h) + v.row_off) * h->d.T_pred; }
int ioc_cluster_exchange(desire_ctx* h, size_t n_groups, bool reset_err, hipStream_t s);
int ioc_cluster_check(desire_ctx* h, hipStream_t s, const char* what);
void ioc_timing_report(const long long* dbg, const char* const* names, int n, hipStream_t s);
int desire_pack_all(desire_ctx* h);
int scene_grad_setup(desire_ctx* h);
inline bool scene_grad_on(const desire_ctx* h) { return h->scene_grad || h->img_set; }
void enc_weights(desire_ctx* h, const char* prefix, EncArgs& e);
IocStepArgs ioc_step_args(desire_ctx* h, int t);
inline RngArgs rng_args(const desire_ctx* h) { return RngArgs{h->rng_state, 0u, 0u, 0u, h->rng_scene_base, h->rng_slot_base}; }
int recon_ws_setup(desire_ctx* h);
int scene_images_run(desire_ctx* h, hipStream_t s);
```

### desire_amd/csrc/ioc_lds.h

```cpp
#pragma once
#include <stddef.h>

#ifdef __HIPCC__
#define IOC_HD __host__ __device__
#else
#define IOC_HD
#endif

template <int N>
struct IocLdsRegions {
    int sz[N] = {};
    IOC_HD constexpr int off(int r) const { int o = 0; for (int i = 0; i < r; ++i) o += sz[i]; return o; }
    IOC_HD constexpr size_t bytes() const { return (size_t)off(N); }
};
#define IOC_LDS_TIED(cond) static_assert(cond, "hand carve-up and ioc_lds.h plan disagree: " #cond)
IOC_HD constexpr int ioc_kx(int H, int EV, int C) { return EV + C + 2 * H; }

constexpr int IOC_POOL_MAX_BINS = 64;
IOC_HD constexpr int ioc_pool_slots(int H, int TM) {
    return 2 * TM - (TM * IOC_POOL_MAX_BINS + (H + 4) * 4 - 1) / ((H + 4) * 4);
}

struct IocLds : IocLdsRegions<12> {
    enum { XH, AB, MASKS, PC, PP, WV, RED, VLD, OCC, ROWBITS, ROWLIST, SPARE };
// ... 62 lines not shown
        IocHtLds l;
        l.sz[X] = T * (ioc_kx(H, EV, C) + 8) * 2;
        l.sz[RH] = T * (H + 8) * 2;
        l.sz[HT] = H * (T + 8) * 2;
        l.sz[MASKS] = T * (bins + 1) * 8;
        l.tail(H, EV, T, T);
        l.sz[PGV] = split ? 8 : 0;
        l.sz[EX] = split ? WM * NT * 4096 : 0;
        l.sz[EXB] = split && bins <= 32 ? WM * NT * 2048 : 0;
        l.sz[SPARE] = split ? 64 : 56;
        return l;
    }
    IOC_HD static constexpr IocHtLds bf16_cluster(int H, int EV, int C, int bins, int MAXM = 128) {
        IocHtLds l;
        l.sz[X] = 32 * (ioc_kx(H, EV, C) + 8) * 2;
        l.sz[RH] = 32 * (H + 8) * 2;
        l.sz[HT] = H * (MAXM + 8) * 2;
        l.sz[MASKS] = 32 * (bins + 1) * 16;
        l.tail(H, EV, 32, MAXM);
        l.sz[PGV] = MAXM * 8;
        l.sz[SPARE] = 64;
        return l;
    }
    IOC_HD static constexpr IocHtLds x3(int H, int EV, int C, int NP, int bins) {
        IocHtLds l;
        l.sz[X] = NP * 32 * (ioc_kx(H, EV, C) + 8) * 2;
        l.sz[RH] = NP * 32 * (H + 8) * 2;
        l.sz[HT] = NP * H * (32 + 8) * 2;
        l.sz[MASKS] = ((32 * (bins + 1) + 1) & ~1) * 4;
        l.tail(H, EV, 32, 32);
        l.sz[SPARE] = 8;
        return l;
    }
    IOC_HD static constexpr IocHtLds x6r2(int H, int EV, int C, int bins) {
        IocHtLds l;
        l.sz[X] = 64 * (ioc_kx(H, EV, C) + 4) * 4;
        l.sz[RH] = 64 * (H + 4) * 4;
        l.sz[HT] = H * (64 + 4) * 4;
        l.sz[MASKS] = 64 * (bins + 1) * 8;
        l.tail(H, EV, 64, 64);
        l.sz[SPARE] = 56;
        return l;
    }
};

struct IocBwdLds : IocLdsRegions<14> {
    enum { A1, A2, A3, MASKS, OBS, PC, DSC, WSC, VLD, OCC, ROWBITS, ROWLIST, LUT, SPARE };
    IOC_HD constexpr void common(int H, int T, int bins, int mw, int M) {
        sz[A1] = T * (H + 4) * 4;
        sz[A2] = 2 * T * (H + 4) * 4;
        sz[MASKS] = T * bins * mw;
        sz[OBS] = T * bins * mw;
        sz[PC] = M * 8;
        sz[DSC] = T * 4;
        sz[WSC] = H * 4;
        sz[VLD] = M;
        sz[OCC] = 8;
    }
    IOC_HD static constexpr IocBwdLds tile(int H, int TM, int bins) {
        IocBwdLds l;
        l.common(H, TM, bins, TM == 32 ? 4 : 8, TM);
        l.sz[A3] = TM * (H + 4) * 4;
        l.sz[ROWBITS] = 36 * 4;
        l.sz[ROWLIST] = TM == 32 && H <= 128 ? (H / 32) * 32 : 0;
        l.sz[SPARE] = 424 - l.sz[ROWLIST];
        return l;
    }
    IOC_HD static constexpr IocBwdLds x3(int H, int bins) {
        IocBwdLds l;
        l.common(H, 32, bins, 4, 32);
        l.sz[A3] = 2 * 32 * (H + 8) * 2;
        l.sz[LUT] = 16 * 8;
        l.sz[SPARE] = 56;
        return l;
    }
    IOC_HD static constexpr IocBwdLds cluster(int H, int bins, int MAXM = 128) {
        IocBwdLds l;
        l.common(H, 32, bins, 16, MAXM);
        l.sz[A3] = MAXM * (H + 4) * 4;
        l.sz[SPARE] = 64;
        return l;
    }
};
```

### desire_amd/csrc/ioc_plan.h

```cpp
#pragma once
#include "../../include/desire_hip.h"
#include "ioc_lds.h"

#include <functional>

inline bool ioc_uses_cluster(int mno, int H, int bins, int variant) {
    if (mno > 64 || (mno == 64 && H == 256) || (variant == 4 && mno >= 64)) return true;
    return mno == 64 && IocLds::tile(H, 16, 32, 64, bins).bytes() > 160 * 1024;
}
inline int ioc_bin_split(long R, int mno, int H, int bins, int iters) {
    if (mno > 32 || H > 128 || iters != 1) return 1;
    const long tiles = (R + 31) / 32;
    for (int n = 4; n >= 2; --n)
        if (tiles * n <= 256 && bins >= n) return n;
    return 1;
}
inline bool ioc_x3_supported(int mno, int H, int bins) { return mno >= 1 && mno <= 32 && 32 % mno == 0 && (H == 64 || H == 128) && bins <= 64; }
inline bool ioc_x6r2_supported(int mno, int H, int bins) {
    if (!((H == 64 || H == 128) && mno >= 1 && ((mno <= 32 && 32 % mno == 0) || mno == 64))) return false;
    return IocHtLds::x6r2(H, 16, 32, bins).bytes() <= 160 * 1024;
}
inline bool ioc_bwd_x3_supported(int mno, int H) { return mno <= 32 && (H == 64 || H == 128); }

enum class IocFwd { STEPWISE, FP32, FP32_WIDE, FP32_CLUSTER, BF16, BF16_WIDE, BF16_CLUSTER, X3, X3R2, X6, X6R2 };
enum class IocBwd { FP32, X3, CLUSTER };

struct IocPlan {
    IocFwd fwd = IocFwd::FP32;
    int nspl = 1;
    IocBwd bwd = IocBwd::FP32;
    bool padded = false;
    bool cluster() const { return fwd == IocFwd::FP32_CLUSTER || fwd == IocFwd::BF16_CLUSTER; }
    bool fp32_weights() const { return fwd == IocFwd::FP32 || fwd == IocFwd::FP32_WIDE || fwd == IocFwd::FP32_CLUSTER; }
};

inline IocPlan ioc_plan(const desire_dims& d, bool training, int mno, int gpt, long R, const std::function<int(int)>& capacity = {}) {
    IocPlan p;
    const int H = d.H, B = d.grid_size * d.grid_size, v = d.ioc_form;
    p.padded = v == DESIRE_IOC_AUTO && H <= 128 && (d.bf16 == 0 || d.bf16 == 2) && (!training || d.bf16 == 0 || !(d.train_fp32_mask & 4));
    p.bwd = ioc_uses_cluster(mno, H, B, 0) ? IocBwd::CLUSTER
          : d.bf16 == 2 && !(d.train_fp32_mask & 4) && ioc_bwd_x3_supported(mno, H) ? IocBwd::X3 : IocBwd::FP32;
    const bool split_mode = (d.bf16 == 2 || d.bf16 == 3) && !training;
    const bool split_served = ioc_x3_supported(d.mno, H, B) || (d.mno == 64 && ioc_x6r2_supported(d.mno, H, B));
    if (d.mno > 128 || (split_mode && !split_served && H == 256 && v == DESIRE_IOC_AUTO)) { p.fwd = IocFwd::STEPWISE; return p; }
    const bool wide64 = mno == 64 && !training && ioc_x6r2_supported(mno, H, B);
    const bool x3 = d.bf16 == 2 && (ioc_x3_supported(mno, H, B) || wide64 || (gpt > 0 && ioc_x3_supported(32, H, B)));
    const bool x6 = d.bf16 == 3 && (ioc_x3_supported(mno, H, B) || wide64);
    const bool cluster = d.bf16 == 1 ? (mno > 64 || (mno == 64 && (v == DESIRE_IOC_CLUSTER || v == DESIRE_IOC_CLUSTER_BINS)))
                                     : (!(x3 || x6) || training) && ioc_uses_cluster(mno, H, B, v);
    const bool wide = mno > 32 || v == DESIRE_IOC_TILE64;
    const IocFwd fp32 = cluster ? IocFwd::FP32_CLUSTER : wide && H != 256 ? IocFwd::FP32_WIDE : IocFwd::FP32;
    if (training && d.bf16 != 1) p.fwd = x3 ? IocFwd::X3 : fp32;
    else if (x6)
        p.fwd = (mno > 32 || (v != DESIRE_IOC_X6_TILE32 && ((R + 63) / 64 >= 256 || v == DESIRE_IOC_X6_TILE64))) && ioc_x6r2_supported(mno, H, B) ? IocFwd::X6R2 : IocFwd::X6;
    else if (x3)
        p.fwd = mno > 32 && ioc_x6r2_supported(mno, H, B) ? IocFwd::X3R2 : IocFwd::X3;
    else if (d.bf16 == 1) p.fwd = cluster ? IocFwd::BF16_CLUSTER : wide ? IocFwd::BF16_WIDE : IocFwd::BF16;
    else p.fwd = fp32;
    if (p.fwd == IocFwd::FP32 && d.bf16 == 0 && !training && d.ioc_split != 1 && v == DESIRE_IOC_AUTO && gpt == 0 && capacity) {
        int n = ioc_bin_split(R, mno, H, B, d.iters);
        if (n > 1 && d.ioc_split > 1) n = n < d.ioc_split ? n : d.ioc_split;
        const long tiles = (R + 31) / 32;
        while (n > 1 && (long)capacity(n) < tiles * n) --n;
        p.nspl = n;
    }
    return p;
}
```

### desire_amd/csrc/ioc_tile.h

```cpp
#pragma once
#include "ioc_lds.h"

constexpr int IOC_ROW_ZERO = -1, IOC_ROW_SUM = -2;
IOC_HD constexpr int ioc_row_source(unsigned m) { return m == 0u ? IOC_ROW_ZERO : (m & (m - 1u)) ? IOC_ROW_SUM : __builtin_ctz(m); }
IOC_HD constexpr int ioc_row_source(unsigned long long m) { return m == 0ull ? IOC_ROW_ZERO : (m & (m - 1ull)) ? IOC_ROW_SUM : __builtin_ctzll(m); }
IOC_HD constexpr int ioc_row_offset(int code, int TM, int LDX, int E, int LDB, int lane15) {
    return code * (code <= TM ? LDX : LDB) + (code < TM ? E : code == TM ? 4 * lane15 : (TM + 1) * (LDX - LDB));
}

#ifdef __HIPCC__
#include "common.h"

#ifdef DESIRE_IOC_TIMING
#define IOC_TICK(k) { const long long now_ = clock64(); tacc[k] += now_ - tprev; tprev = now_; }
#else
#define IOC_TICK(k)
#endif

template <int EV, int NTHR>
__device__ __forceinline__ void ioc_stage_wv(float* wv, const float* __restrict__ w_vel, const float* __restrict__ b_vel, int tid) {
    for (int i = tid; i < 3 * EV; i += NTHR) wv[i] = (i < 2 * EV) ? w_vel[i] : b_vel[i - 2 * EV];
}
__device__ __forceinline__ void ioc_stage_lut(uint2* lut, int tid) {
    if (tid < 16) {
        const unsigned lo = ((tid & 1) ? 0x3F80u : 0u) | ((tid & 2) ? 0x3F800000u : 0u);
        const unsigned hi2 = ((tid & 4) ? 0x3F80u : 0u) | ((tid & 8) ? 0x3F800000u : 0u);
        lut[tid] = make_uint2(lo, hi2);
    }
}
__device__ __forceinline__ unsigned long long ioc_occ64(const unsigned* occ) {
    unsigned long long om = (unsigned long long)__builtin_amdgcn_readfirstlane((int)occ[0]) & 0xffffffffull;
    om |= (unsigned long long)(unsigned)__builtin_amdgcn_readfirstlane((int)occ[1]) << 32;
    return om;
}
__device__ __forceinline__ float ioc_sum32(float v) {
    v += __shfl_xor(v, 1); v += __shfl_xor(v, 2); v += __shfl_xor(v, 4); v += __shfl_xor(v, 8); v += __shfl_xor(v, 16);
    return v;
}
#endif
```

### desire_amd/csrc/kernels.h

```cpp
#pragma once
#include <hip/hip_runtime.h>
#include <stdint.h>

#include "dyn_count.h"
#include "eval_lds.h"
#include "ioc_lds.h"

template <auto K>
inline const void* big_lds_kernel() {
    static const hipError_t once = hipFuncSetAttribute(reinterpret_cast<const void*>(K), hipFuncAttributeMaxDynamicSharedMemorySize, 160 * 1024);
    (void)once;
    return reinterpret_cast<const void*>(K);
}
template <auto K, class... Args>
inline void launch_big_lds(dim3 grid, dim3 block, size_t lds, hipStream_t s, const Args&... args) {
    (void)big_lds_kernel<K>();
    hipLaunchKernelGGL(K, grid, block, lds, s, args...);
}


enum { EPI_BIAS = 0, EPI_BIAS_RELU = 1, EPI_SCALE_SHIFT_ELU = 2, EPI_NONE = 3, EPI_ELUGRAD = 4, EPI_SIGGRAD = 5 };

struct GemmArgs {
    const float* A; int lda; int M; int K;
// ... 33 lines not shown
};
void launch_mask(const MaskArgs& a, hipStream_t s);
void launch_deconv1_x6(const GemmArgs& a, hipStream_t s);
void launch_mask_x6(const MaskArgs& a, hipStream_t s);

struct ConvArgs {
    const float* in; float* out; int n;
    const float4* Wp; const float* w_raw;
    const float* scale; const float* shift;
    int mode; const float* yprev;
    DynCount dyn;
};
void launch_conv1(const ConvArgs& a, hipStream_t s);
void launch_conv2(const ConvArgs& a, hipStream_t s);
void launch_conv2_x3(const ConvArgs& a, hipStream_t s);
void launch_conv3_x3(const ConvArgs& a, hipStream_t s);
void launch_conv3(const ConvArgs& a, hipStream_t s);
void launch_deconv2(const ConvArgs& a, hipStream_t s);
void launch_deconv3(const ConvArgs& a, hipStream_t s);
void launch_deconv4(const ConvArgs& a, hipStream_t s);

struct EncArgs {
    const float* frames; int n_scenes; int T; int mno;
    float sx, sy; int H;
    const float* wx_g; const float* b_g;
    const float* wx_c; const float* b_c;
    const float4* Whg; const float4* Whc;
    float* out; int ldo;
    float* p_last;
    uint8_t* valid;
    float* sv_r; float* sv_u; float* sv_c; float* sv_h; float* sv_x;
    int n_roll; const float* w5; const float* b5;
    const float* normals; float* roll_out;
    DynCount dyn;
};
void launch_encoder(const EncArgs& a, hipStream_t s);
void launch_encoder_pair(const EncArgs& past, const EncArgs& fut, hipStream_t s);
void launch_encoder_bf16(const EncArgs& a, hipStream_t s);

struct RollArgs {
    const float* h_T; int R; int K; int mno; int H; int T;
    const float* wx_g; const float* b_g; const float* wx_c; const float* b_c; const float4* Whg; const float4* Whc;
    const float* w5; const float* b5;
    const float* normals; RngArgs g;
    float* Y;
};
void launch_rollout_samples(const RollArgs& a, hipStream_t s);
void launch_rollout_normals(const RngArgs& g, float* out, int R, int T, int K, int mno, hipStream_t s);

struct DecArgs {
    const float* xz; const float* Hx; int ldhx; const float* p_last;
    int R; int K; int mno; int H; int T;
    const float4* Wxg; const float4* Wxc; const float4* Whg; const float4* Whc;
    const float* b_g; const float* b_c;
    const float* w_head; const float* b_head;
    float* Y;
    float* hdump;
    float* sv_r; float* sv_u; float* sv_c;
    DynCount dyn;
};
void launch_decoder(const DecArgs& a, hipStream_t s);
void launch_decoder_bf16(const DecArgs& a, hipStream_t s);

struct IocArgs {
    float* Y; float* score;
    const float* Hx; int ldhx; const float* p_last; const uint8_t* valid;
    int R; int K; int mno; int H; int T; int iters;
    int C; int Gh; int Gw; int E_v; int G; float nb_w, nb_h;
    const float* grids; const int32_t* grid_of_scene;
    const float* w_vel; const float* b_vel;
    const float4* Wsoc; const float* b_soc;
    const float4* Wsoc_c;
    const float4* Wg; const float4* Wc; const float* b_g; const float* b_c;
    const float* w_score; const float* b_score;
    const float4* Wreg; const float* b_reg; int NTreg;
    int variant;
    long long* dbg;
    float* hex; int* grp_cnt; int* err;
    int nspl;
    float* sv_x; float* sv_r; float* sv_u; float* sv_c; float* sv_h;
    const float* bin_tab;
    int gpt; int ngrp;
    DynCount dyn;
};
void launch_ioc(const IocArgs& a, bool wide, hipStream_t s);
void launch_ioc_cluster(const IocArgs& a, hipStream_t s);
int ioc_bin_split_capacity(const IocArgs& a, int n);
void launch_ioc_bf16(const IocArgs& a, bool wide, hipStream_t s);
int launch_ioc_bf16_cluster(const IocArgs& a, hipStream_t s);
void launch_ioc_x3(const IocArgs& a, hipStream_t s);
void launch_ioc_x6(const IocArgs& a, hipStream_t s);
void launch_ioc_x6r2(const IocArgs& a, hipStream_t s);
void launch_ioc_x3r2(const IocArgs& a, hipStream_t s);
void launch_decoder_x6(const DecArgs& a, hipStream_t s, int np = 3);
void launch_deconv2_x6(const ConvArgs& a, hipStream_t s, int np = 3);
void launch_deconv3_x6(const ConvArgs& a, hipStream_t s, int np = 3);
struct IocStepArgs {
    int t; int rank; int nranks; int m_loc; int n_scenes; int K; int R;
    int H; int T; int Gh; int Gw; int G; float nb_w, nb_h;
    const float* Yall; const float* plast_all; const uint8_t* valid_all; const float* Hall;
    int peer; const float* Yp[8]; const float* plp[8]; const uint8_t* vp[8]; const float* Hp[8];
    const float* st_h; float* st_h_out; float* st_score; float* st_h_copy;
    const float* grids; const int32_t* grid_of_scene;
    const float* w_vel; const float* b_vel; const float4* Wsoc; const float* b_soc;
    const float4* Wg; const float4* Wc; const float* b_g; const float* b_c; const float* w_score;
    const float* bin_tab;
    int np; size_t plo_soc, plo_g, plo_c;
};
void launch_ioc_step(const IocStepArgs& a, hipStream_t s);
struct PeerFlags { const unsigned* f[8]; };
void launch_peer_wait(const PeerFlags& flags, int nranks, const unsigned* epoch, unsigned per_pass, unsigned stage, int* err, hipStream_t s);
void launch_peer_set(unsigned* flag, const unsigned* epoch, unsigned per_pass, unsigned stage, hipStream_t s);
void launch_peer_epoch(unsigned* epoch, hipStream_t s);
void launch_hx_rows(float* out, const float* HxHy, int ldhx, int n_scenes, int K, int mno, int H, hipStream_t s);
void launch_peer_publish(const uint8_t* valid, const float* p_last, const float* Y, const float* HxHy, int ldhx, uint8_t* o_valid,
                         float* o_plast, float* o_Y, float* o_H, int n_scenes, int K, int mno, int T, int H, hipStream_t s);
void launch_ioc_finish(float* Y, const float* dY, const float* st_score, const float* b_score, float* score, int R, int T, hipStream_t s);
struct ConvArgs;
void launch_deconv2_bf16(const ConvArgs& a, hipStream_t s);
void launch_conv2_bf16(const ConvArgs& a, hipStream_t s);
void launch_conv3_bf16(const ConvArgs& a, hipStream_t s);
void launch_deconv1_bf16(const GemmArgs& a, hipStream_t s);
void launch_mask_bf16(const MaskArgs& a, hipStream_t s);
void launch_deconv3_bf16(const ConvArgs& a, hipStream_t s);
void launch_deconv34_bf16(const ConvArgs& a, const float* sc4, const float* sh4, hipStream_t s);

void launch_neighbor_bins(const float* pos, const uint8_t* valid, int32_t* bins, int n_groups, int mno,
                          float nb_w, float nb_h, int G, const float* bin_tab, hipStream_t s);
void launch_scene_cells(const float* pos, int32_t* cells, int n, int Gh, int Gw, hipStream_t s);

void launch_fill_f32(float* dst, size_t n, float v, hipStream_t s);
void launch_copy_f32(float* dst, const float* src, size_t n, hipStream_t s);
void launch_copy_cols(float* dst, const float* src, size_t rows, int cols, int ld, hipStream_t s);
void launch_instnorm_act(float* x, int n, int P, int C, const float* gamma, const float* beta, int sig, hipStream_t s);
void launch_instnorm_act_oop(const float* x, float* y, int n, int P, int C, const float* gamma, const float* beta, int sig, hipStream_t s);
void launch_instnorm_act_bwd(float* dy, const float* x, const float* y, int n, int P, int C, const float* gamma, int sig, hipStream_t s);
void launch_batchnorm_act(float* x, size_t n, int P, int C, const float* gamma, const float* beta, int sig, float* part, float* stat, hipStream_t s);
void launch_batchnorm_act_bwd(float* dy, const float* x, const float* y, size_t n, int P, int C, const float* gamma, int sig,
                              float* part, float* stat, float* stat2, hipStream_t s);
void launch_conv_direct(const float* in, const float* w, const float* b, float* out, int n, int Hi, int Wi, int Ci,
                        int Co, int stride, int relu, hipStream_t s);
void launch_temporal_conv(const float* frames, const float* w, const float* b, float* rho, int n_scenes, int T, int mno,
                          hipStream_t s);
void launch_feature_pooling(const float* Y, const float* rho, float* out, int R, int T, int K, int mno, hipStream_t s);
void launch_losses(const float* params, const float* Y, const float* fut, const uint8_t* lmask, const float* nfut, float* kld,
                   float* recon, float* cost, int n_scenes, int mno, int K, int T, int L, float sx, float sy, hipStream_t s);
void launch_loss_mask(const uint8_t* valid, const float* fut, uint8_t* lmask, float* nfut, int n_scenes, int mno, int T, hipStream_t s);
void launch_build_windows(const float* frames, int F, int mno_in, const int32_t* starts, int n, int T_obs, int T_pred,
                          int mno, float* past, float* fut, int32_t* err, int lookahead, hipStream_t s);
void launch_gaussian_sample(const float* p, const float* nrm, float* out, int n, hipStream_t s);
void launch_ade_fde(const float* Y, const float* fut, float* out, int n_scenes, int mno, int K, int T, float sx, float sy,
                    hipStream_t s);

struct RankHz { int n; int h[8]; };
constexpr int RANK_MAX_K = 4096;
void launch_rank_select(const float* score, const float* Y, int32_t* order, float* top_Y, float* top_score, int n_scenes, int mno, int K,
                        int T, int n_top, hipStream_t s);
void launch_ranked_errors(const float* Y, const float* fut, const int32_t* order, float* tab, int32_t* cnt, float* out, int n_scenes, int mno,
                          int K, int T, int n_top, const RankHz& hz, float sx, float sy, float ux, float uy, hipStream_t s);

void launch_sample_errors(const float* Y, const float* fut, float* tab, int32_t* cnt, int n_scenes, int mno, int K, int T, const RankHz& hz,
                          float sx, float sy, float ux, float uy, hipStream_t s);

void launch_kde_nll(const float* Y, const float* fut, const float* score, float* w, float* st, float* out, float* frame, int n_scenes, int mno,
                    int K, int T, const RankHz& hz, float sx, float sy, float ux, float uy, float log_floor, hipStream_t s);

void launch_select_diverse(const float* Y, const int32_t* order, const float* score, int32_t* order_out, int32_t* count, float* mass, float* top_Y,
                           float* top_score, int n_scenes, int mno, int K, int T, int metric, int t_end, int n_top, float radius, float ux,
// ... 123 lines not shown
```

### desire_amd/csrc/kernels_rnn.hip

```cpp
#include "common.h"
#include "kernels.h"
#include <cstdlib>
#include <map>
#include <tuple>

#define RNN_WG 512

__device__ __forceinline__ f32x16 splat16(float v) {
    f32x16 z;
#pragma unroll
    for (int i = 0; i < 16; ++i) z[i] = v;
    return z;
}

__device__ __forceinline__ void mma1(f32x16& acc, const float* a_lane, const float4* __restrict__ b_lane, int G) {
    f32x16 t[1] = {acc};
    mma_groups<1>(t, a_lane, 0, b_lane, G);
    acc = t[0];
}

template <int H, int TM, bool ROLL>
__device__ __forceinline__ void encoder_tile(const EncArgs& a, int blk) {
    extern __shared__ __attribute__((aligned(16))) float smem[];
    constexpr int LDH = H + 4, NT = H >> 5, G = H >> 3, NTHR = NT * (TM / 32) * 64;
// ... 278 lines not shown
                const int rl = mt * 32 + acc_row(i);
                if (SAVE && a.hdump && row0 + rl < a.R) a.hdump[sv_t + (sv_lane + ((i & 3) + 8 * (i >> 2)) * sv_row)] = h[i];
            }
        }
        __syncthreads();
        {
            const int r = tid / TPR;
            float s0 = 0.f, s1 = 0.f;
#pragma unroll
            for (int jj = 0; jj < 4; ++jj) {
                const float4 hv = *reinterpret_cast<const float4*>(hs + r * LDH + hq * 16 + 4 * ((jj + hrot) & 3));
                s0 = fmaf(hv.x, hw0[4 * jj], s0); s1 = fmaf(hv.x, hw1[4 * jj], s1);
                s0 = fmaf(hv.y, hw0[4 * jj + 1], s0); s1 = fmaf(hv.y, hw1[4 * jj + 1], s1);
                s0 = fmaf(hv.z, hw0[4 * jj + 2], s0); s1 = fmaf(hv.z, hw1[4 * jj + 2], s1);
                s0 = fmaf(hv.w, hw0[4 * jj + 3], s0); s1 = fmaf(hv.w, hw1[4 * jj + 3], s1);
            }
            const int q8 = hq;
            s0 += __shfl_xor(s0, 1); s1 += __shfl_xor(s1, 1);
            s0 += __shfl_xor(s0, 2); s1 += __shfl_xor(s1, 2);
            if (TPR >= 8) { s0 += __shfl_xor(s0, 4); s1 += __shfl_xor(s1, 4); }
            if (TPR >= 16) { s0 += __shfl_xor(s0, 8); s1 += __shfl_xor(s1, 8); }
            if (q8 == 0 && row0 + r < a.R) {
                float2 y = make_float2(pl[r * 2] + (s0 + bh0), pl[r * 2 + 1] + (s1 + bh1));
                *reinterpret_cast<float2*>(a.Y + ((size_t)(row0 + r) * a.T + t) * 2) = y;
            }
        }
    }
}
template <int H, int TM>
static void launch_decoder_t(const DecArgs& a, hipStream_t s) {
    const size_t lds = (2 * TM * (H + 4) + 2 * H + TM * 2) * sizeof(float);
    if (a.sv_r || a.sv_c || a.hdump) {
        launch_big_lds<k_decoder<H, TM, true>>(dim3((a.R + TM - 1) / TM), dim3((H / 32) * (TM / 32) * 64), lds, s, a);
    } else {
        launch_big_lds<k_decoder<H, TM, false>>(dim3((a.R + TM - 1) / TM), dim3((H / 32) * (TM / 32) * 64), lds, s, a);
    }
}
void launch_decoder(const DecArgs& a, hipStream_t s) {
    if (a.H == 256) launch_decoder_t<256, 32>(a, s);
    else if (a.H == 128) {
        launch_decoder_t<128, 32>(a, s);
    }
    else launch_decoder_t<64, 64>(a, s);
}

#include "cluster.h"
#include "ioc_tile.h"
#include "split.h"
template <int TM> struct MaskT { typedef unsigned long long type; };
template <> struct MaskT<32> { typedef unsigned type; };
__device__ __forceinline__ int ffs_(unsigned m) { return __ffs((int)m); }
__device__ __forceinline__ int ffs_(unsigned long long m) { return __ffsll((long long)m); }
typedef float f32x4v __attribute__((ext_vector_type(4)));
template <int G>
__device__ __forceinline__ void ioc_bin_chain(f32x16& acc, const float* a_lane, const float4* __restrict__ b_lane, float4 (&b0)[4]) {
    static_assert(G % 8 == 0, "whole pairs of chunks");
    float4 b1[4];
    float4 an = *reinterpret_cast<const float4*>(a_lane);
    auto chunk = [&](int g0, const float4 (&b)[4]) {
#pragma unroll
        for (int j = 0; j < 4; ++j) {
            const float4 av = an;
            if (g0 + j + 1 < G) an = *reinterpret_cast<const float4*>(a_lane + (g0 + j + 1) * 8);
            __builtin_amdgcn_sched_barrier(0);
            acc = mfma32(av.x, b[j].x, acc);
            acc = mfma32(av.y, b[j].y, acc);
            acc = mfma32(av.z, b[j].z, acc);
            acc = mfma32(av.w, b[j].w, acc);
            __builtin_amdgcn_sched_barrier(0);
        }
    };
#pragma unroll
    for (int c = 0; c < G / 4; c += 2) {
        load_b4(b1, b_lane, 4 * c + 4);
        __builtin_amdgcn_sched_barrier(0);
        chunk(4 * c, b0);
        __builtin_amdgcn_sched_barrier(0);
        if (c + 2 < G / 4) load_b4(b0, b_lane, 4 * c + 8);
        __builtin_amdgcn_sched_barrier(0);
        chunk(4 * c + 4, b1);
        __builtin_amdgcn_sched_barrier(0);
    }
}
template <int H, int EV, int C, int TM, bool TRAIN, bool CP = false, int NSPL = 1, bool PAD = false>
__global__ __launch_bounds__((H / 32) * (TM / 32) * 64, ((H / 32) * (TM / 32) <= 2) ? 1 : 2) void k_ioc(IocArgs a) {
#ifdef DESIRE_IOC_TIMING
    long long tacc[10] = {0, 0, 0, 0, 0, 0, 0, 0, 0, 0};
    long long tprev = clock64();
#endif
    extern __shared__ __attribute__((aligned(16))) float smem[];
    constexpr int NT = H >> 5, E = EV + C + H, KX = E + H, LDX = KX + 4, LDB = H + 4;
    constexpr int NTHR = NT * (TM / 32) * 64, TPR = NTHR / TM;
    constexpr int G8 = KX >> 3, GH = H >> 3;
    constexpr int NCH = H / (4 * TPR);
    const int B = a.G * a.G;
    float* XH = smem;
    float* AB = XH + (TM + 1) * LDX;
    typedef typename MaskT<TM>::type mask_t;
    mask_t* masks = reinterpret_cast<mask_t*>(AB + 2 * TM * LDB);
    float* pc = reinterpret_cast<float*>(masks + TM * B);
    float* pp = pc + TM * 2;
    float* wv = pp + TM * 2;
    float* red = wv + 3 * EV;
    unsigned char* vld = reinterpret_cast<unsigned char*>(red + NT * TM);
    unsigned* occ = reinterpret_cast<unsigned*>(vld + TM);
    unsigned* rowbits = occ + 2;
    unsigned* rowlist = rowbits + 36;
    constexpr IocLds P0 = IocLds::tile(H, EV, C, TM, 0), P1 = IocLds::tile(H, EV, C, TM, 1);
    IOC_LDS_TIED(P0.off(P0.MASKS) == ((TM + 1) * LDX + 2 * TM * LDB) * 4);
    IOC_LDS_TIED(P0.sz[P0.MASKS] == 0 && P1.sz[P1.MASKS] == TM * (int)sizeof(mask_t));
    IOC_LDS_TIED(P0.off(P0.ROWLIST) - P0.off(P0.PC) == (TM * 2 * 2 + 3 * EV + NT * TM) * 4 + TM + (2 + 36) * 4);
    IOC_LDS_TIED(P0.sz[P0.ROWLIST] == 2 * (TM / 4) * 4);
    constexpr bool INPLACE = !CP && !(TM == 64 && ((H == 128 && TRAIN) || (H == 64 && !TRAIN)));
    constexpr int NSLOT = ioc_pool_slots(H, TM);
    unsigned char* rsrc = reinterpret_cast<unsigned char*>(AB + NSLOT * LDB);
    unsigned* nsum = rowbits;
    IOC_LDS_TIED(NSLOT > 0 && (2 * TM - NSLOT) * LDB * 4 >= TM * IOC_POOL_MAX_BINS && 3 * TM < 256 && P0.sz[P0.ROWBITS] >= 4);
    static_assert(LDX % 4 == 0 && LDB % 4 == 0 && E % 4 == 0 && 4 * 15 + 4 + 8 * (GH - 1) + 4 <= LDX, "16-byte units; the zero row holds a slot per lane");

    const int lane = lane_id(), w = wave_id(), tid = threadIdx.x;
    const int cb = w % NT, mt = w / NT;
    const int tile = NSPL > 1 ? (int)blockIdx.x / NSPL : (int)blockIdx.x, member = NSPL > 1 ? (int)blockIdx.x % NSPL : 0;
    const int row0 = tile * TM;
    IOC_DYN(a)
    if (a.dyn.cnt && row0 >= a.R) return;
    unsigned long long my_bins = ~0ull;
    if (NSPL > 1) { my_bins = 0ull; for (int b = member; b < 64; b += NSPL) my_bins |= 1ull << b; }
    const bool active = cb < NT;
    const int col = cb * 32 + (lane & 31);
    const int r8 = tid / TPR, q8 = tid % TPR;
    const int my_row = min(row0 + r8, a.R - 1);
    const int gpt = PAD ? a.gpt : 0;
    const bool dead_row = gpt && (r8 / a.mno >= gpt || tile * gpt + r8 / a.mno >= a.ngrp);
    const int my_scene = gpt ? min(tile * gpt + min(r8 / a.mno, gpt - 1), a.ngrp - 1) / a.K : my_row / (a.K * a.mno);
    const int grp_base = (r8 / a.mno) * a.mno;
    const int my_slot = r8 - grp_base;
    const int n_nb = dead_row ? 0 : a.mno;

    ioc_stage_wv<EV, NTHR>(wv, a.w_vel, a.b_vel, tid);
    for (int i = tid; i < LDX; i += NTHR) XH[TM * LDX + i] = 0.f;
    if (tid < TM) { const int ag = ioc_agent_of_row(min(row0 + tid, a.R - 1), a.K, a.mno, gpt, a.ngrp); vld[tid] = ag >= 0 ? a.valid[ag] : 0; }

    float bgr = 0, bgu = 0, bcc = 0, bso = 0, wsc = 0;
    if (active) { bgr = a.b_g[col]; bgu = a.b_g[H + col]; bcc = a.b_c[col]; bso = a.b_soc[col]; wsc = a.w_score[col]; }
    const float* x_lane = XH + (mt * 32 + (lane & 31)) * LDX + 4 * (lane >> 5);
    float* my_x = XH + (mt * 32 + 4 * (lane >> 5)) * LDX + col;
    const float* grid = a.grids + (size_t)a.grid_of_scene[my_scene] * a.Gh * a.Gw * C;
    const size_t sv_tb = TRAIN ? (size_t)row0 * a.T * H : 0;
    float* sv_r_t = TRAIN ? a.sv_r + sv_tb : nullptr; float* sv_u_t = TRAIN ? a.sv_u + sv_tb : nullptr;
    float* sv_c_t = TRAIN ? a.sv_c + sv_tb : nullptr; float* sv_h_t = TRAIN ? a.sv_h + sv_tb : nullptr;
    auto sv_off = [&](int i, int t) { return (unsigned)(((mt * 32 + 4 * (lane >> 5) + (i & 3) + 8 * (i >> 2)) * a.T + t) * H + col); };

    constexpr int NS = 2;
    auto build = [&](int b, int buf) {
        float* ab = AB + buf * TM * LDB + r8 * LDB;
        mask_t m2 = masks[r8 * B + b];
        int off[NS];
#pragma unroll
        for (int sl = 0; sl < NS; ++sl) {
            off[sl] = m2 ? (grp_base + ffs_(m2) - 1) * LDX : TM * LDX;
            m2 &= m2 - 1;
        }
        float4 s[NCH];
#pragma unroll
        for (int c = 0; c < NCH; ++c) {
            const float4 v0 = *reinterpret_cast<const float4*>(XH + off[0] + E + q8 * 4 + c * 4 * TPR);
            const float4 v1 = *reinterpret_cast<const float4*>(XH + off[1] + E + q8 * 4 + c * 4 * TPR);
            s[c].x = v0.x + v1.x; s[c].y = v0.y + v1.y; s[c].z = v0.z + v1.z; s[c].w = v0.w + v1.w;
        }
        if (__any(m2 != 0)) {
            while (m2) {
                const int j = ffs_(m2) - 1;
                m2 &= m2 - 1;
                const float* src = XH + (grp_base + j) * LDX + E + q8 * 4;
#pragma unroll
                for (int c = 0; c < NCH; ++c) {
                    const float4 v = *reinterpret_cast<const float4*>(src + c * 4 * TPR);
                    s[c].x += v.x; s[c].y += v.y; s[c].z += v.z; s[c].w += v.w;
                }
            }
        }
#pragma unroll
        for (int c = 0; c < NCH; ++c) *reinterpret_cast<float4*>(ab + q8 * 4 + c * 4 * TPR) = s[c];
    };
    auto pool_rows = [&](unsigned long long om) {
        int r = r8, q = q8, gb = grp_base;
        asm volatile("" : "+v"(r), "+v"(q), "+v"(gb));
        unsigned mlo = 0u, mhi = 0u;
        for (int b = q; b < B; b += TPR) {
            const int src = ioc_row_source(masks[r * B + b]);
            if (src == IOC_ROW_SUM) { if (b < 32) mlo |= 1u << b; else mhi |= 1u << (b - 32); }
            else rsrc[r * B + b] = (unsigned char)(src == IOC_ROW_ZERO ? TM : gb + src);
        }
#pragma unroll
        for (int d = 1; d < TPR; d <<= 1) { mlo |= __shfl_xor(mlo, d); if (B > 32) mhi |= __shfl_xor(mhi, d); }
        unsigned long long multi = (((unsigned long long)mhi << 32) | mlo) & om;
        while (multi) {
            const int b = ffs_(multi) - 1;
            multi &= multi - 1;
            int slot = 0;
            if (q == 0) slot = (int)atomicAdd(nsum, 1u);
            slot = __shfl(slot, lane & ~(TPR - 1));
            if (slot >= NSLOT) continue;
            mask_t m2 = masks[r * B + b];
            const float* s0 = XH + (gb + ffs_(m2) - 1) * LDX + E + q * 4;
            m2 &= m2 - 1;
            const float* s1 = XH + (gb + ffs_(m2) - 1) * LDX + E + q * 4;
            m2 &= m2 - 1;
            float4 s[NCH];
#pragma unroll
            for (int c = 0; c < NCH; ++c) {
                const float4 v0 = *reinterpret_cast<const float4*>(s0 + c * 4 * TPR);
                const float4 v1 = *reinterpret_cast<const float4*>(s1 + c * 4 * TPR);
                s[c].x = v0.x + v1.x; s[c].y = v0.y + v1.y; s[c].z = v0.z + v1.z; s[c].w = v0.w + v1.w;
            }
            while (m2) {
                const float* src = XH + (gb + ffs_(m2) - 1) * LDX + E + q * 4;
                m2 &= m2 - 1;
#pragma unroll
                for (int c = 0; c < NCH; ++c) {
                    const float4 v = *reinterpret_cast<const float4*>(src + c * 4 * TPR);
                    s[c].x += v.x; s[c].y += v.y; s[c].z += v.z; s[c].w += v.w;
                }
            }
#pragma unroll
            for (int c = 0; c < NCH; ++c) *reinterpret_cast<float4*>(AB + slot * LDB + q * 4 + c * 4 * TPR) = s[c];
            if (q == 0) rsrc[r * B + b] = (unsigned char)(TM + 1 + slot);
        }
    };

    for (int it = 0; it < a.iters; ++it) {
        for (int i = tid; i < TM * (H >> 2); i += NTHR) {
            const int r = i / (H >> 2), c4 = i - r * (H >> 2);
            const int ag = ioc_agent_of_row(min(row0 + r, a.R - 1), a.K, a.mno, gpt, a.ngrp);
            *reinterpret_cast<float4*>(XH + r * LDX + E + c4 * 4) =
                ag >= 0 ? *reinterpret_cast<const float4*>(a.Hx + (size_t)ag * a.ldhx + c4 * 4) : make_float4(0.f, 0.f, 0.f, 0.f);
        }
        if (tid < TM) {
            const int ag = ioc_agent_of_row(min(row0 + tid, a.R - 1), a.K, a.mno, gpt, a.ngrp);
            pp[tid * 2] = ag >= 0 ? a.p_last[(size_t)ag * 2] : 0.f;
            pp[tid * 2 + 1] = ag >= 0 ? a.p_last[(size_t)ag * 2 + 1] : 0.f;
        }
        __syncthreads();
        f32x16 h = zero16(), sp = zero16();
        if (active) {
#pragma unroll
            for (int i = 0; i < 16; ++i) h[i] = my_x[((i & 3) + 8 * (i >> 2)) * LDX + E];
        }

        float2 ynext = make_float2(0.f, 0.f);
        if (tid < TM) {
            const float2 y0 = *reinterpret_cast<const float2*>(a.Y + ((size_t)min(row0 + tid, a.R - 1) * a.T) * 2);
            pc[tid * 2] = y0.x; pc[tid * 2 + 1] = y0.y;
        }
        for (int i = tid; i < TM * B; i += NTHR) masks[i] = 0;
        if (tid < 2) occ[tid] = 0;
        if (INPLACE && tid == 2) *nsum = 0;
        if (CP && tid < B) rowbits[tid] = 0;
        __syncthreads();
        const float* rh_lane = AB + (mt * 32 + (lane & 31)) * LDB + 4 * (lane >> 5);
        float* my_rh = AB + (mt * 32 + 4 * (lane >> 5)) * LDB + col;
        constexpr int GX = E >> 3;

        for (int t = 0; t < a.T; ++t) {
            IOC_TICK(0)
            if (tid < TM && t + 1 < a.T)
                ynext = *reinterpret_cast<const float2*>(a.Y + ((size_t)min(row0 + tid, a.R - 1) * a.T + t + 1) * 2);
            {
                const float px = pc[r8 * 2], py = pc[r8 * 2 + 1];
                const float vx = px - pp[r8 * 2], vy = py - pp[r8 * 2 + 1];
                constexpr int per = EV / TPR;
#pragma unroll
                for (int j = q8 * per; j < (q8 + 1) * per; ++j)
                    XH[r8 * LDX + j] = fmaxf(fmaf(vy, wv[EV + j], vx * wv[j]) + wv[2 * EV + j], 0.f);
                int cy, cx;
                scene_cell_dev(px, py, a.Gh, a.Gw, cy, cx);
                const float* gsrc = grid + ((size_t)cy * a.Gw + cx) * C;
                constexpr int cper = C / TPR;
                if (cper >= 4) {
#pragma unroll
                    for (int j = q8 * cper; j < (q8 + 1) * cper; j += 4)
                        *reinterpret_cast<float4*>(XH + r8 * LDX + EV + j) = *reinterpret_cast<const float4*>(gsrc + j);
                } else {
                    *reinterpret_cast<float2*>(XH + r8 * LDX + EV + q8 * 2) = *reinterpret_cast<const float2*>(gsrc + q8 * 2);
                }
                float nbw, nbh;
                nb_opaque(a.nb_w, a.nb_h, nbw, nbh);
                const unsigned long long oc = nb_search<4>(pc, vld, grp_base, n_nb, q8, TPR, my_slot, px, py, nbw, nbh, a.G, a.bin_tab,
                                                          [&](int j, int b) {
                                                              atomicOr(&masks[r8 * B + b], (mask_t)1 << j);
                                                              if (CP) atomicOr(&rowbits[b], 1u << r8);
                                                          });
                nb_publish_occ(oc, occ, B);
                if (CP) {
#pragma unroll
                    for (int c = 0; c < NCH; ++c)
                        *reinterpret_cast<float4*>(XH + r8 * LDX + EV + C + q8 * 4 + c * 4 * TPR) = make_float4(0.f, 0.f, 0.f, 0.f);
                }
            }
            __syncthreads();
            IOC_TICK(1)
            if constexpr (CP) {
                unsigned long long om = ioc_occ64(occ);
                constexpr int T16 = H / 16;
                auto build_c = [&](int b, int buf) {
                    const unsigned rb = rowbits[b];
                    if (!((rb >> r8) & 1u)) return;
                    const int slot = __popc(rb & ((1u << r8) - 1u));
                    float* ab = AB + buf * TM * LDB + slot * LDB;
                    mask_t m2 = masks[r8 * B + b];
                    const int o0 = (grp_base + ffs_(m2) - 1) * LDX;
                    m2 &= m2 - 1;
                    const int o1 = m2 ? (grp_base + ffs_(m2) - 1) * LDX : TM * LDX;
                    m2 &= m2 - 1;
                    float4 sacc[NCH];
#pragma unroll
                    for (int c = 0; c < NCH; ++c) {
                        const float4 v0 = *reinterpret_cast<const float4*>(XH + o0 + E + q8 * 4 + c * 4 * TPR);
                        const float4 v1 = *reinterpret_cast<const float4*>(XH + o1 + E + q8 * 4 + c * 4 * TPR);
                        sacc[c].x = v0.x + v1.x; sacc[c].y = v0.y + v1.y; sacc[c].z = v0.z + v1.z; sacc[c].w = v0.w + v1.w;
                    }
                    while (m2) {
                        const int j = ffs_(m2) - 1;
                        m2 &= m2 - 1;
                        const float* src = XH + (grp_base + j) * LDX + E + q8 * 4;
#pragma unroll
                        for (int c = 0; c < NCH; ++c) {
                            const float4 v = *reinterpret_cast<const float4*>(src + c * 4 * TPR);
                            sacc[c].x += v.x; sacc[c].y += v.y; sacc[c].z += v.z; sacc[c].w += v.w;
                        }
                    }
#pragma unroll
                    for (int c = 0; c < NCH; ++c) *reinterpret_cast<float4*>(ab + q8 * 4 + c * 4 * TPR) = sacc[c];
                    if (q8 == 0) reinterpret_cast<unsigned char*>(rowlist + buf * (TM / 4))[slot] = (unsigned char)r8;
                };
                int buf = 0;
                if (om) build_c(ffs_(om) - 1, 0);
                __syncthreads();
                while (om) {
                    const int b = ffs_(om) - 1;
                    om &= om - 1;
                    const float4* w0 = a.Wsoc_c + ((size_t)(b * T16 + 2 * cb) * T16) * 64 + lane;
                    float4 wf[2][T16];
                    if (active) {
#pragma unroll
                        for (int g = 0; g < T16; ++g) { wf[0][g] = w0[g * 64]; wf[1][g] = w0[(T16 + g) * 64]; }
                    }
                    if (om) build_c(ffs_(om) - 1, buf ^ 1);
                    const int nrows = __popc(__builtin_amdgcn_readfirstlane((int)rowbits[b]));
                    if (active) {
                        for (int c16 = 0; c16 * 16 < nrows; ++c16) {
                            f32x4v a0 = {0.f, 0.f, 0.f, 0.f}, a1 = {0.f, 0.f, 0.f, 0.f};
                            const float* ap = AB + buf * TM * LDB + (16 * c16 + (lane & 15)) * LDB + 4 * (lane >> 4);
#pragma unroll
                            for (int g = 0; g < T16; ++g) {
                                const float4 av = *reinterpret_cast<const float4*>(ap + 16 * g);
                                a0 = __builtin_amdgcn_mfma_f32_16x16x4f32(av.x, wf[0][g].x, a0, 0, 0, 0);
                                a1 = __builtin_amdgcn_mfma_f32_16x16x4f32(av.x, wf[1][g].x, a1, 0, 0, 0);
                                a0 = __builtin_amdgcn_mfma_f32_16x16x4f32(av.y, wf[0][g].y, a0, 0, 0, 0);
                                a1 = __builtin_amdgcn_mfma_f32_16x16x4f32(av.y, wf[1][g].y, a1, 0, 0, 0);
                                a0 = __builtin_amdgcn_mfma_f32_16x16x4f32(av.z, wf[0][g].z, a0, 0, 0, 0);
                                a1 = __builtin_amdgcn_mfma_f32_16x16x4f32(av.z, wf[1][g].z, a1, 0, 0, 0);
                                a0 = __builtin_amdgcn_mfma_f32_16x16x4f32(av.w, wf[0][g].w, a0, 0, 0, 0);
                                a1 = __builtin_amdgcn_mfma_f32_16x16x4f32(av.w, wf[1][g].w, a1, 0, 0, 0);
                            }
                            const unsigned rl4 = rowlist[buf * (TM / 4) + 4 * c16 + (lane >> 4)];
                            float* ex = XH + EV + C + cb * 32 + (lane & 15);
#pragma unroll
                            for (int i = 0; i < 4; ++i) {
                                if (16 * c16 + 4 * (lane >> 4) + i < nrows) {
                                    float* dst = ex + ((rl4 >> (8 * i)) & 0xffu) * LDX;
                                    dst[0] += a0[i];
                                    dst[16] += a1[i];
                                }
                            }
                        }
                    }
                    __syncthreads();
                    buf ^= 1;
                }
                if (active) {
#pragma unroll
                    for (int i = 0; i < 16; ++i) {
                        float* e = my_x + ((i & 3) + 8 * (i >> 2)) * LDX + EV + C;
                        *e = fmaxf(*e + bso, 0.f);
                    }
                }
            } else
            {
                f32x16 soc = zero16();
                unsigned long long om = ioc_occ64(occ);
                if (NSPL > 1) om &= my_bins;
                int buf = 0;
                bool in_place = false;
                if constexpr (INPLACE) {
                    if (om) pool_rows(om);
                    __syncthreads();
                    in_place = __builtin_amdgcn_readfirstlane((int)*nsum) <= NSLOT;
                } else {
                    if (om) build(ffs_(om) - 1, 0);
                    __syncthreads();
                }
                IOC_TICK(2)
                if (INPLACE && !in_place) {
                    if (om) build(ffs_(om) - 1, 0);
                    __syncthreads();
                }
                __builtin_amdgcn_s_setprio(3);
                if (INPLACE && in_place) {
                    int ln = lane;
                    asm volatile("" : "+v"(ln));
                    const unsigned char* my_src = rsrc + (mt * 32 + (ln & 31)) * B;
                    const float* a0 = smem + 4 * (ln >> 5);
                    if (om && active) {
                        int code = my_src[ffs_(om) - 1];
                        while (om) {
                            const int b = ffs_(om) - 1;
                            om &= om - 1;
                            const float4* wb = a.Wsoc + ((size_t)(b * NT + cb) * GH) * 64 + lane;
                            float4 wb0[4];
                            load_b4(wb0, wb, 0);
                            const float* ap = a0 + ioc_row_offset(code, TM, LDX, E, LDB, ln & 15);
                            code = my_src[om ? ffs_(om) - 1 : b];
                            __builtin_amdgcn_sched_barrier(0);
                            ioc_bin_chain<GH>(soc, ap, wb, wb0);
                        }
                    }
                    IOC_TICK(4)
                    om = 0;
                }
                while (om) {
                    const int b = ffs_(om) - 1;
                    om &= om - 1;
                    const float4* wb = a.Wsoc + ((size_t)(b * NT + cb) * GH) * 64 + lane;
                    float4 wb0[4];
                    if (active) load_b4(wb0, wb, 0);
                    if (om) build(ffs_(om) - 1, buf ^ 1);
                    IOC_TICK(3)
                    if (active) ioc_bin_chain<GH>(soc, AB + buf * TM * LDB + (mt * 32 + (lane & 31)) * LDB + 4 * (lane >> 5), wb, wb0);
                    IOC_TICK(4)
                    __syncthreads();
                    IOC_TICK(5)
                    buf ^= 1;
                }
                __builtin_amdgcn_s_setprio(0);
                if constexpr (NSPL > 1) {
                    const int sidx = it * a.T + t;
                    float* slot = a.hex + (((size_t)tile * 2 + (sidx & 1)) * NSPL) * (TM * H);
                    uint2* mine = reinterpret_cast<uint2*>(slot + (size_t)member * TM * H) + (size_t)w * 8 * 64 + lane;
#pragma unroll
                    for (int q = 0; q < 8; ++q) st_agent_u64(mine + q * 64, make_uint2(__float_as_uint(soc[2 * q]), __float_as_uint(soc[2 * q + 1])));
                    group_publish_wt(a.grp_cnt + tile);
                    group_wait_wt(a.grp_cnt + tile, NSPL * (sidx + 1), a.err);
                    f32x16 tot = zero16();
#pragma unroll
                    for (int m = 0; m < NSPL; ++m) {
                        if (m == member) {
#pragma unroll
                            for (int i = 0; i < 16; ++i) tot[i] += soc[i];
                        } else {
                            const uint2* src = reinterpret_cast<const uint2*>(slot + (size_t)m * TM * H) + (size_t)w * 8 * 64 + lane;
#pragma unroll
                            for (int q = 0; q < 8; ++q) {
                                const uint2 v = ld_agent_u64(src + q * 64);
                                tot[2 * q] += __uint_as_float(v.x); tot[2 * q + 1] += __uint_as_float(v.y);
                            }
                        }
                    }
                    soc = tot;
                }
                if (active) {
#pragma unroll
                    for (int i = 0; i < 16; ++i) my_x[((i & 3) + 8 * (i >> 2)) * LDX + EV + C] = fmaxf(soc[i] + bso, 0.f);
                }
            }
            __syncthreads();
            IOC_TICK(6)
            if (TRAIN) {
                for (int i = tid; i < TM * (E >> 2); i += NTHR) {
                    const int r = i / (E >> 2), c4 = i - r * (E >> 2);
                    if (row0 + r < a.R)
                        *reinterpret_cast<float4*>(a.sv_x + ((size_t)(row0 + r) * a.T + t) * E + c4 * 4) =
                            *reinterpret_cast<const float4*>(XH + r * LDX + c4 * 4);
                }
            }
            __builtin_amdgcn_s_setprio(2);
            f32x16 rh, u;
            if (active) {
                rh = zero16(); u = zero16();
                mma1(rh, x_lane, a.Wg + ((size_t)cb * G8) * 64 + lane, G8);
                mma1(u, x_lane, a.Wg + ((size_t)(cb + NT) * G8) * 64 + lane, G8);
#pragma unroll
                for (int i = 0; i < 16; ++i) {
                    const float r = sigmoidf_(rh[i] + bgr);
                    if (TRAIN && row0 + mt * 32 + acc_row(i) < a.R) sv_r_t[sv_off(i, t)] = r;
                    rh[i] = r * h[i];
                }
#pragma unroll
                for (int i = 0; i < 16; ++i) my_rh[((i & 3) + 8 * (i >> 2)) * LDB] = rh[i];
#pragma unroll
                for (int i = 0; i < 16; ++i) {
                    u[i] = sigmoidf_(u[i] + bgu);
                    if (TRAIN && row0 + mt * 32 + acc_row(i) < a.R) sv_u_t[sv_off(i, t)] = u[i];
                }
            }
            __syncthreads();
            IOC_TICK(7)
            if (active) {
                f32x16 ac = zero16();
                mma1(ac, x_lane, a.Wc + ((size_t)cb * G8) * 64 + lane, GX);
                mma1(ac, rh_lane, a.Wc + ((size_t)cb * G8 + GX) * 64 + lane, GH);
#pragma unroll
                for (int i = 0; i < 16; ++i) {
                    const float c = tanhf_(ac[i] + bcc);
                    h[i] = gru_blend(u[i], h[i], c);
                    sp[i] = fmaf(h[i], wsc, sp[i]);
                    if (TRAIN && row0 + mt * 32 + acc_row(i) < a.R) { sv_c_t[sv_off(i, t)] = c; sv_h_t[sv_off(i, t)] = h[i]; }
                }
#pragma unroll
                for (int i = 0; i < 16; ++i)
                    my_x[((i & 3) + 8 * (i >> 2)) * LDX + E] = h[i];
            }
            __builtin_amdgcn_s_setprio(0);
            if (tid < TM) {
                pp[tid * 2] = pc[tid * 2]; pp[tid * 2 + 1] = pc[tid * 2 + 1];
                pc[tid * 2] = ynext.x; pc[tid * 2 + 1] = ynext.y;
            }
            for (int i = tid; i < TM * B; i += NTHR) masks[i] = 0;
            if (tid < 2) occ[tid] = 0;
            if (INPLACE && tid == 2) *nsum = 0;
            if (CP && tid < B) rowbits[tid] = 0;
            __syncthreads();
            IOC_TICK(8)
        }
#pragma unroll
        for (int i = 0; i < 16; ++i) {
            float v = active ? sp[i] : 0.f;
            v = ioc_sum32(v);
            if ((lane & 31) == 0) red[cb * TM + mt * 32 + acc_row(i)] = v;
        }
        __syncthreads();
        bool poisoned = false;
        if constexpr (NSPL > 1) poisoned = __hip_atomic_load(a.err, __ATOMIC_RELAXED, __HIP_MEMORY_SCOPE_SYSTEM) != 0;
        if (tid < TM && row0 + tid < a.R && it == a.iters - 1 && member == 0) {
            float sc = 0.f;
#pragma unroll
            for (int c = 0; c < NT; ++c) sc += red[c * TM + tid];
            a.score[row0 + tid] = poisoned ? __builtin_nanf("") : sc + (float)a.T * a.b_score[0];
        }
        for (int nt = cb; nt < a.NTreg; nt += NT) {
            f32x16 acc = zero16();
            mma1(acc, x_lane + E, a.Wreg + ((size_t)nt * GH) * 64 + lane, GH);
            const int cc = nt * 32 + (lane & 31);
            if (cc < 2 * a.T) {
                const float bb = a.b_reg[cc];
#pragma unroll
                for (int i = 0; i < 16; ++i) {
                    const int row = row0 + mt * 32 + acc_row(i);
                    if (row < a.R && member == 0) {
                        float* y = a.Y + (size_t)row * 2 * a.T + cc;
                        *y = poisoned ? __builtin_nanf("") : *y + (acc[i] + bb);
                    }
                }
            }
        }
        __syncthreads();
    }
#ifdef DESIRE_IOC_TIMING
    if (a.dbg && tile == 7 && member == 0 && tid == 0)
        for (int k = 0; k < 10; ++k) a.dbg[k] = tacc[k];
#endif
}
template <int H, int TM>
static void launch_ioc_t(const IocArgs& a, hipStream_t s) {
    const dim3 grid((a.R + TM - 1) / TM), block((H / 32) * (TM / 32) * 64);
    const size_t lds = IocLds::tile(H, 16, 32, TM, a.G * a.G).bytes();
    if (a.sv_h) {
        if constexpr (TM == 32 && H <= 128) {
            if (a.gpt > 0) {
                launch_big_lds<k_ioc<H, 16, 32, 32, true, true, 1, true>>(grid, block, lds, s, a);
                return;
            }
        }
        if constexpr (TM == 32 && H <= 128) {
            if (a.variant != 9) {
                launch_big_lds<k_ioc<H, 16, 32, 32, true, true>>(grid, block, lds, s, a);
                return;
            }
        }
        if constexpr (H <= 128 || TM == 32) {
            launch_big_lds<k_ioc<H, 16, 32, TM, true>>(grid, block, lds, s, a);
        }
        return;
    }
    if constexpr (TM == 32 && H <= 128) {
        if (a.variant == 8) {
            launch_big_lds<k_ioc<H, 16, 32, 32, false, true>>(grid, block, lds, s, a);
            return;
        }
    }
    if constexpr (TM == 32 && H <= 128) {
        if (a.nspl > 1) {
            const dim3 gs(grid.x * a.nspl);
            switch (a.nspl) {
                case 3: launch_big_lds<k_ioc<H, 16, 32, 32, false, false, 3>>(gs, block, lds, s, a); return;
                case 4: launch_big_lds<k_ioc<H, 16, 32, 32, false, false, 4>>(gs, block, lds, s, a); return;
                default: launch_big_lds<k_ioc<H, 16, 32, 32, false, false, 2>>(gs, block, lds, s, a); return;
            }
        }
    }
    if constexpr (TM == 32 && H <= 128) {
        if (a.gpt > 0) {
            launch_big_lds<k_ioc<H, 16, 32, 32, false, false, 1, true>>(grid, block, lds, s, a);
            return;
        }
    }
    launch_big_lds<k_ioc<H, 16, 32, TM, false>>(grid, block, lds, s, a);
}
template <int H>
static const void* bin_split_kernel(int n) {
    return n == 2 ? big_lds_kernel<k_ioc<H, 16, 32, 32, false, false, 2>>() : n == 3 ? big_lds_kernel<k_ioc<H, 16, 32, 32, false, false, 3>>()
                                                                                     : big_lds_kernel<k_ioc<H, 16, 32, 32, false, false, 4>>();
}
int ioc_bin_split_capacity(const IocArgs& a, int n) {
    if (a.mno > 32 || a.H > 128 || n < 2 || n > 4) return 0;
    static std::map<std::tuple<int, int, int, size_t>, int> cache;
    int dev = 0;
    if (hipGetDevice(&dev) != hipSuccess) return 0;
    const size_t lds = IocLds::tile(a.H, 16, 32, 32, a.G * a.G).bytes();
    const auto key = std::make_tuple(dev, a.H, n, lds);
    auto it = cache.find(key);
    if (it != cache.end()) return it->second;
    const void* kern = a.H == 128 ? bin_split_kernel<128>(n) : bin_split_kernel<64>(n);
    int per_cu = 0, cus = 0;
    int cap = 0;
    if (hipOccupancyMaxActiveBlocksPerMultiprocessor(&per_cu, kern, (a.H / 32) * 64, lds) == hipSuccess && per_cu > 0 &&
        hipDeviceGetAttribute(&cus, hipDeviceAttributeMultiprocessorCount, dev) == hipSuccess)
        cap = per_cu * cus;
    cache[key] = cap;
    return cap;
}
void launch_ioc(const IocArgs& a, bool wide, hipStream_t s) {
    if (a.H == 256) launch_ioc_t<256, 32>(a, s);
    else if (a.H == 128) { if (wide) launch_ioc_t<128, 64>(a, s); else launch_ioc_t<128, 32>(a, s); }
    else { if (wide) launch_ioc_t<64, 64>(a, s); else launch_ioc_t<64, 32>(a, s); }
}

template <int H, int EV, int C, bool TRAIN = false>
__global__ __launch_bounds__((H / 32) * 64, (H / 32) <= 4 ? 1 : 2) void k_ioc_cl(IocArgs a) {
    extern __shared__ __attribute__((aligned(16))) float smem[];
    constexpr int TM = 32, MAXM = 128;
    constexpr int NT = H >> 5, E = EV + C + H, KX = E + H, LDX = KX + 4, LDB = H + 4;
    constexpr int NTHR = NT * 64, TPR = NTHR / TM;
    constexpr int G8 = KX >> 3, GH = H >> 3, GX = E >> 3;
    constexpr int NCH = H / (4 * TPR);
    const int B = a.G * a.G;
    const int tpg = a.mno / 32;
    float* XH = smem;
    float* AB = XH + TM * LDX;
    unsigned long long* masks = reinterpret_cast<unsigned long long*>(AB + 2 * TM * LDB);
    float* pg = reinterpret_cast<float*>(masks + TM * B * 2);
    float* pp = pg + MAXM * 2;
    float* wv = pp + TM * 2;
    float* red = wv + 3 * EV;
    unsigned char* vld = reinterpret_cast<unsigned char*>(red + NT * TM);
    unsigned* occ = reinterpret_cast<unsigned*>(vld + MAXM);
    constexpr IocLds P0 = IocLds::cluster(H, EV, C, 0, MAXM), P1 = IocLds::cluster(H, EV, C, 1, MAXM);
    IOC_LDS_TIED(P0.off(P0.MASKS) == (TM * LDX + 2 * TM * LDB) * 4);
    IOC_LDS_TIED(P0.sz[P0.MASKS] == 0 && P1.sz[P1.MASKS] == TM * 2 * 8);
    IOC_LDS_TIED(P0.off(P0.OCC) - P0.off(P0.PC) == (MAXM * 2 + TM * 2 + 3 * EV + NT * TM) * 4 + MAXM);

    const int lane = lane_id(), w = wave_id(), tid = threadIdx.x;
    const int cb = w;
    const int col = cb * 32 + (lane & 31);
    const int r8 = tid / TPR, q8 = tid % TPR;
    const int tile_pos = blockIdx.x % tpg;
    IOC_DYN(a)
    const int n_tiles = a.R / TM;

    ioc_stage_wv<EV, NTHR>(wv, a.w_vel, a.b_vel, tid);
    const float bgr = a.b_g[col], bgu = a.b_g[H + col], bcc = a.b_c[col], bso = a.b_soc[col], wsc = a.w_score[col];
    const float* x_lane = XH + (lane & 31) * LDX + 4 * (lane >> 5);
    float* my_x = XH + (4 * (lane >> 5)) * LDX + col;
    const float* rh_lane = AB + (lane & 31) * LDB + 4 * (lane >> 5);
    float* my_rh = AB + (4 * (lane >> 5)) * LDB + col;
    int epoch = 0;

    for (int tile = blockIdx.x; tile < n_tiles; tile += gridDim.x) {
        const int row0 = tile * TM;
        const int grow0 = row0 - tile_pos * TM;
        const int group = grow0 / a.mno;
        int* cnt = a.grp_cnt + group;
        const int scene = grow0 / (a.K * a.mno);
        const float* grid = a.grids + (size_t)a.grid_of_scene[scene] * a.Gh * a.Gw * C;
        const int my_slot = tile_pos * TM + r8;
        int base = 0;
// ... 798 lines not shown
```

### desire_amd/spec.py

```python
from __future__ import annotations

import dataclasses
from dataclasses import dataclass
from typing import Dict, Tuple

import numpy as np

BN_EPS = 1e-3


IOC_AUTO, IOC_TILE64, IOC_CLUSTER, IOC_CLUSTER_BINS, IOC_COMPACT, IOC_TRAIN_DENSE, IOC_X6_TILE32, IOC_X6_TILE64 = 0, 2, 4, 6, 8, 9, 13, 14
FLAG_NO_FUSE34 = 1
FLAG_COMPACT_ROWS = 4
FLAG_COMPACT_IOC = 8
FLAG_TRAIN_FWD_3P = 2


@dataclass(frozen=True)
class Dims:

    n_scenes: int = 1
    mno: int = 32
    K: int = 20
    T_obs: int = 8
    T_pred: int = 40
    H: int = 128
    L: int = 128
    S: int = 32
    C: int = 32
    Gh: int = 64
    Gw: int = 64
    n_grids: int = 1
    grid_size: int = 4
    E_v: int = 16
    iters: int = 1
    posterior: int = 1
    nb_w: float = 0.25
    nb_h: float = 0.25
    sx: float = 1.0
    sy: float = 1.0
    bin_mode: int = 0
    bn_mode: int = 0
    bf16: int = 0
    ref_compat: int = 0
    n_dec: int = 0
    ioc_form: int = 0
    ioc_split: int = 0
    train_fp32_mask: int = 0
    flags: int = 0

    @property
    def A(self) -> int:
        return self.n_scenes * self.mno

    @property
    def R(self) -> int:
        return self.A * self.K

    @property
    def V(self) -> int:
        return self.S * self.S

    @property
    def B(self) -> int:
        return self.grid_size * self.grid_size

    @property
    def E(self) -> int:
        return self.E_v + self.C + self.H

    def validate(self) -> None:
        if self.S != 32:
            raise ValueError("CVAE stack closes only for S=32 (rnn_size=512), model/model.py:465-468")
        if not (1 <= self.mno <= 256) or (32 % self.mno if self.mno <= 32 else self.mno % 32):
            raise ValueError("mno must divide 32 or be a multiple of 32 up to 256 (host pads max_num_obj up; above 128: inference only)")
        if self.mno > 128 and self.bf16 == 1:
            raise ValueError("more than 128 agents per scene run the fp32 step-wise IOC (bf16 = 0, 2 or 3)")
        if self.L % 8 or self.C % 8 or self.E_v % 8:
            raise ValueError("L%8, C%8, E_v%8 required by the MFMA tiling")
        if self.H not in (16, 32, 64, 128, 256):
            raise ValueError("H must be 16, 32 (run zero-padded on the 64-wide recurrent tile), 64, 128 or 256")
        if self.ref_compat:
            if not (self.K == 1 and self.posterior and self.bn_mode == 1 and not self.bf16 and self.n_dec >= 1
                    and self.H == 2 * self.T_obs and self.T_pred == self.T_obs):
                raise ValueError("ref_compat (model/model.py:116-311): K=1, posterior, bn_mode=1, fp32, H == 2*T_obs, T_pred == T_obs, n_dec >= 1")
        elif self.n_dec:
            raise ValueError("n_dec belongs to ref_compat")
        if self.C != 32 or self.E_v != 16:
            raise ValueError("C=32, E_v=16 are the instantiated IOC widths in this round")
        if min(self.n_scenes, self.K, self.T_obs, self.T_pred, self.n_grids, self.iters) < 1:
            raise ValueError("sizes must be >= 1")

    def replace(self, **kw) -> "Dims":
        return dataclasses.replace(self, **kw)


def ioc_pool_slots(H: int, TM: int) -> int:
    row = (H + 4) * 4
# ... 111 lines not shown
```

### include/desire_hip.h

```cpp
#ifndef DESIRE_HIP_H
#define DESIRE_HIP_H

#include <stddef.h>
#include <stdint.h>

#ifdef __cplusplus
extern "C" {
#endif

#define DESIRE_OK 0
#define DESIRE_ERR_ARG (-1)
#define DESIRE_ERR_STATE (-2)
#define DESIRE_ERR_HIP (-3)
#define DESIRE_ERR_NODEV (-4)

typedef struct desire_dims {
    int32_t n_scenes, mno, K, T_obs, T_pred;
    int32_t H, L, S, C, Gh, Gw, n_grids;
    int32_t grid_size, E_v, iters, posterior;
    float nb_w, nb_h, sx, sy;
    int32_t bin_mode;
    int32_t bn_mode;
    int32_t bf16;
    int32_t ref_compat;
    int32_t n_dec;
    int32_t ioc_form;
    int32_t ioc_split;
    int32_t train_fp32_mask;
    int32_t flags;
} desire_dims;

#define DESIRE_IOC_AUTO 0
#define DESIRE_IOC_TILE64 2
#define DESIRE_IOC_CLUSTER 4
#define DESIRE_IOC_CLUSTER_BINS 6
#define DESIRE_IOC_COMPACT 8
#define DESIRE_IOC_TRAIN_DENSE 9
#define DESIRE_IOC_X6_TILE32 13
#define DESIRE_IOC_X6_TILE64 14
#define DESIRE_FLAG_NO_FUSE34 1
#define DESIRE_FLAG_TRAIN_FWD_3P 2

#define DESIRE_FLAG_COMPACT_ROWS 4

#define DESIRE_FLAG_COMPACT_IOC 8

typedef struct desire_ctx desire_handle;

const char* desire_last_error(void);
int desire_version(void);
int desire_dims_size(void);
const char* desire_build_hash(void);
int desire_set_option(desire_handle* h, const char* name, int32_t value);

int desire_create(const desire_dims* dims, desire_handle** out);
int desire_destroy(desire_handle* h);

int desire_set_weight(desire_handle* h, const char* name, const float* host_data, size_t n);
int desire_finalize_weights(desire_handle* h);

int desire_set_scene_grids(desire_handle* h, const float* dev_grids, const int32_t* host_grid_of_scene);
int desire_set_scene_images(desire_handle* h, const float* dev_images, int32_t Hi, int32_t Wi, const int32_t* host_grid_of_scene);

int desire_encode(desire_handle* h, const float* dev_past, const float* dev_fut, void* stream);

int desire_sample(desire_handle* h, const float* dev_eps, float* dev_Yhat, void* stream);

int desire_ioc_refine(desire_handle* h, float* dev_Yhat, float* dev_score, void* stream);

int desire_forward(desire_handle* h, const float* dev_past, const float* dev_fut, const float* dev_eps,
                   float* dev_Yhat, float* dev_score, void* stream);

int desire_set_rng(desire_handle* h, uint64_t seed, uint32_t draw, void* stream);
int desire_set_rng_origin(desire_handle* h, uint32_t scene_base, uint32_t slot_base);
int desire_rng_state(desire_handle* h, uint32_t host_out[2], void* stream);
#define DESIRE_RNG_BITS 0
#define DESIRE_RNG_NORMAL 1
#define DESIRE_RNG_LATENT 2
#define DESIRE_RNG_ROLLOUT 3
int desire_rng_fill(desire_handle* h, uint64_t seed, uint32_t stream_id, uint64_t first, int32_t kind, void* dev_out, size_t n, void* stream);

int desire_read_buffer(desire_handle* h, const char* name, float* host_out, size_t n, void* stream);

int desire_get_bin_table(desire_handle* h, float* host_out20);
int desire_neighbor_bins(desire_handle* h, const float* dev_pos, const uint8_t* dev_valid,
                         int32_t* dev_bins, int32_t n_groups, void* stream);
int desire_scene_cells(desire_handle* h, const float* dev_pos, int32_t* dev_cells, int32_t n, void* stream);

int desire_scene_cnn(desire_handle* h, const float* dev_image, int32_t Hi, int32_t Wi, float* dev_grids, void* stream);

int desire_losses(desire_handle* h, const float* dev_fut, const float* dev_Yhat, float* dev_kld, float* dev_recon,
                  float* dev_cost, void* stream);

int desire_temporal_conv(desire_handle* h, const float* dev_past, float* dev_rho, void* stream);
int desire_feature_pooling(desire_handle* h, const float* dev_Yhat, const float* dev_rho, float* dev_out, void* stream);

int desire_build_windows(desire_handle* h, const float* dev_frames, int32_t n_frames, int32_t mno_in,
                         const int32_t* host_starts, int32_t n_windows, float* dev_past, float* dev_fut, void* stream);
int desire_build_windows_la(desire_handle* h, const float* dev_frames, int32_t n_frames, int32_t mno_in,
                          const int32_t* host_starts, int32_t n_windows, int32_t lookahead, float* dev_past, float* dev_fut, void* stream);
int desire_gaussian_sample(desire_handle* h, const float* dev_params, const float* dev_normals, float* dev_out,
                           int32_t n, void* stream);
int desire_rollout(desire_handle* h, const float* dev_past, const float* dev_normals, int32_t num, float* dev_out, void* stream);
int desire_rollout_samples(desire_handle* h, const float* dev_past, const float* dev_normals, float* dev_Yhat, void* stream);
int desire_ade_fde(desire_handle* h, const float* dev_Yhat, const float* dev_fut, float* dev_out, void* stream);

int desire_rank_samples(desire_handle* h, const float* dev_score, const float* dev_Yhat, int32_t n_top,
                        int32_t* dev_order, float* dev_top_Y, float* dev_top_score, void* stream);
int desire_ranked_errors(desire_handle* h, const float* dev_Yhat, const float* dev_fut, const int32_t* dev_order, int32_t n_top,
                         const int32_t* host_horizons, int32_t n_h, float unit_x, float unit_y, float* dev_out, void* stream);

#define DESIRE_KDE_MIN_DET_RATIO 1e-5f
int desire_kde_nll(desire_handle* h, const float* dev_Yhat, const float* dev_fut, const float* dev_score, const int32_t* host_horizons,
                   int32_t n_h, float unit_x, float unit_y, float log_floor, float* dev_out, float* dev_frame, void* stream);

#define DESIRE_DIST_FINAL 0
#define DESIRE_DIST_MEAN  1
#define DESIRE_DIST_MAX   2
int desire_select_diverse(desire_handle* h, const float* dev_Yhat, const int32_t* dev_order, const float* dev_score,
                          int32_t metric, int32_t t_end, float radius, float unit_x, float unit_y, int32_t n_top,
                          int32_t* dev_order_out, int32_t* dev_count, float* dev_mass,
                          float* dev_top_Y, float* dev_top_score, void* stream);

int desire_joint_metrics(desire_handle* h, const float* dev_Yhat, const float* dev_fut, const uint8_t* dev_present,
                         const float* dev_score, const int32_t* host_horizons, int32_t n_h, int32_t n_top,
                         float radius, float unit_x, float unit_y,
                         int32_t* dev_first, int32_t* dev_cnt, float* dev_jerr, float* dev_jscore, int32_t* dev_jorder,
                         float* dev_out, void* stream);

#define DESIRE_WORLD_ALL  0
// ... 77 lines not shown
```

Baseline: 2.629 million samples/s.

## Add IOC prepass kernel precomputing per-step inputs and neighbor masks

Adds a separate prepass kernel that, for each 32-row tile and time step, precomputes velocity embeddings, scene-grid features, social-pooling neighbor masks, row sources and occupancy into a workspace record. The dense fp32 IOC kernel gains a PRE variant that loads these records, prefetching the next step's record during the GEMM, instead of doing the neighbor search and embedding inline, which drops a barrier per step. It is enabled by default for fp32 inference with a single IOC iteration and no split. The cost is an extra kernel launch, a workspace buffer, and global-memory traffic for the records.

```diff
diff --git a/desire_amd/_build.py b/desire_amd/_build.py
--- a/desire_amd/_build.py
+++ b/desire_amd/_build.py
@@ -9,7 +9,7 @@
 HERE = os.path.dirname(os.path.abspath(__file__))
 CSRC = os.path.join(HERE, "csrc")
 LIB = os.path.join(HERE, "libdesire_hip.so")
-SOURCES = ["api.hip", "api_pack.hip", "api_forward.hip", "api_peer.hip", "api_ops.hip", "kernels_gemm.hip", "kernels_conv.hip", "kernels_rnn.hip", "kernels_aux.hip", "kernels_rank.hip", "kernels_kde.hip", "kernels_select.hip", "kernels_joint.hip", "kernels_worlds.hip", "kernels_plan.hip", "kernels_modes.hip", "kernels_scene_modes.hip", "kernels_occ.hip", "kernels_recon.hip", "kernels_compact.hip", "kernels_bwd.hip", "kernels_bwd_x3.hip", "kernels_bwd_cl.hip", "kernels_bf16.hip", "kernels_bf16_cl.hip", "kernels_x3.hip", "kernels_x6.hip", "kernels_x6r2.hip", "kernels_scene.hip", "kernels_rng.hip", "kernels_rollout.hip", "train.hip", "backward.hip"]
+SOURCES = ["api.hip", "api_pack.hip", "api_forward.hip", "api_peer.hip", "api_ops.hip", "kernels_gemm.hip", "kernels_conv.hip", "kernels_rnn.hip", "kernels_ioc_pre.hip", "kernels_aux.hip", "kernels_rank.hip", "kernels_kde.hip", "kernels_select.hip", "kernels_joint.hip", "kernels_worlds.hip", "kernels_plan.hip", "kernels_modes.hip", "kernels_scene_modes.hip", "kernels_occ.hip", "kernels_recon.hip", "kernels_compact.hip", "kernels_bwd.hip", "kernels_bwd_x3.hip", "kernels_bwd_cl.hip", "kernels_bf16.hip", "kernels_bf16_cl.hip", "kernels_x3.hip", "kernels_x6.hip", "kernels_x6r2.hip", "kernels_scene.hip", "kernels_rng.hip", "kernels_rollout.hip", "train.hip", "backward.hip"]
 FLAGS = ["--offload-arch=gfx950", "-O3", "-std=c++17", "-fPIC", "-Wno-unused-value", "-Wno-pass-failed"]
 FLAGS += os.environ.get("DESIRE_HIPCC_FLAGS", "").split()
 _SINK = ["-mllvm", "-sink-insts-to-avoid-spills"]
diff --git a/desire_amd/_lib.py b/desire_amd/_lib.py
--- a/desire_amd/_lib.py
+++ b/desire_amd/_lib.py
@@ -13,7 +13,7 @@
 EXPORTS = [
     "desire_last_error", "desire_version", "desire_dims_size", "desire_build_hash", "desire_create", "desire_destroy", "desire_set_weight",
     "desire_finalize_weights", "desire_set_scene_grids", "desire_set_scene_images", "desire_encode", "desire_sample",
-    "desire_ioc_refine", "desire_forward", "desire_read_buffer", "desire_neighbor_bins",
+    "desire_ioc_refine", "desire_ioc_plan_info", "desire_forward", "desire_read_buffer", "desire_neighbor_bins",
     "desire_scene_cells", "desire_set_profiling", "desire_get_profile", "desire_scene_cnn", "desire_losses",
     "desire_temporal_conv", "desire_feature_pooling", "desire_build_windows", "desire_gaussian_sample", "desire_ade_fde",
     "desire_set_training", "desire_backward", "desire_get_grad", "desire_grad_buffer",
@@ -143,6 +143,7 @@
     lib.desire_set_rng_origin.argtypes = [vp, C.c_uint32, C.c_uint32]
     lib.desire_rng_state.argtypes = [vp, C.POINTER(C.c_uint32), vp]
     lib.desire_rng_fill.argtypes = [vp, C.c_uint64, C.c_uint32, C.c_uint64, i32, vp, C.c_size_t, vp]
+    lib.desire_ioc_plan_info.argtypes = [vp, C.POINTER(C.c_int32)]
     lib.desire_set_profiling.argtypes = [vp, C.c_int]
     lib.desire_get_profile.argtypes = [vp, C.POINTER(C.c_float), C.POINTER(C.c_char_p), C.POINTER(C.c_int32)]
     for n in EXPORTS:
@@ -500,6 +501,11 @@
         _chk(self.lib.desire_get_weight(self._h, name.encode(), out.ctypes.data_as(C.POINTER(C.c_float)), out.size, stream or None))
         return out
 
+    def ioc_plan_info(self) -> Dict[str, int]:
+        out = (C.c_int32 * 3)()
+        _chk(self.lib.desire_ioc_plan_info(self._h, out))
+        return {"fwd": int(out[0]), "nspl": int(out[1]), "prepass": int(out[2])}
+
     def set_profiling(self, on: bool) -> None:
         _chk(self.lib.desire_set_profiling(self._h, int(on)))
 
diff --git a/desire_amd/csrc/api.hip b/desire_amd/csrc/api.hip
--- a/desire_amd/csrc/api.hip
+++ b/desire_amd/csrc/api.hip
@@ -89,7 +89,7 @@
     }
     if (d.ioc_split < 0 || d.ioc_split > 4) return fail(DESIRE_ERR_ARG, "ioc_split must be 0 (auto), 1 (never split: batch-size invariant results) or 2..4 (cap)");
     if (d.train_fp32_mask < 0 || d.train_fp32_mask > 15) return fail(DESIRE_ERR_ARG, "train_fp32_mask is a mask of bits 1, 2, 4, 8");
-    if (d.flags & ~(DESIRE_FLAG_NO_FUSE34 | DESIRE_FLAG_TRAIN_FWD_3P | DESIRE_FLAG_COMPACT_ROWS | DESIRE_FLAG_COMPACT_IOC)) return fail(DESIRE_ERR_ARG, "unknown bit in flags (DESIRE_FLAG_*)");
+    if (d.flags & ~(DESIRE_FLAG_NO_FUSE34 | DESIRE_FLAG_TRAIN_FWD_3P | DESIRE_FLAG_COMPACT_ROWS | DESIRE_FLAG_COMPACT_IOC | DESIRE_FLAG_IOC_NO_PREPASS)) return fail(DESIRE_ERR_ARG, "unknown bit in flags (DESIRE_FLAG_*)");
     if ((d.flags & DESIRE_FLAG_COMPACT_IOC) && d.ref_compat) return fail(DESIRE_ERR_ARG, "DESIRE_FLAG_COMPACT_IOC: ref_compat has no IOC stage");
     if ((d.flags & DESIRE_FLAG_COMPACT_ROWS) && (d.bn_mode == 2 || d.ref_compat))
         return fail(DESIRE_ERR_ARG, "DESIRE_FLAG_COMPACT_ROWS: not with bn_mode = 2 (whole-batch statistics depend on the padding rows) or ref_compat");
@@ -206,6 +206,7 @@
         {"rank_tab", d.ref_compat ? 0 : R * 16 * f}, {"rank_cnt", d.ref_compat ? 0 : A * 8 * sizeof(int32_t)},
         {"kde_w", d.ref_compat ? 0 : R * f}, {"kde_st", d.ref_compat ? 0 : A * 2 * f},
         {"joint_js", d.ref_compat ? 0 : (size_t)d.n_scenes * d.K * f}, {"joint_je", d.ref_compat ? 0 : (size_t)d.n_scenes * d.K * 16 * f},
+        {"ioc_pre", !d.ref_compat && ioc_prepass_dims(d) ? ioc_pre_bytes((long)R, d.T_pred, d.E_v, d.C, d.grid_size * d.grid_size) : 0},
     };
     if (int rc = ws_ensure(h, list)) { desire_destroy(h); return rc; }
     for (const WsItem& w : list) (void)hipMemset(W(h, w.n), 0, w.bytes);
@@ -379,6 +380,12 @@
     return DESIRE_OK;
 }
 
+extern "C" int desire_ioc_plan_info(desire_handle* h, int32_t* out3) {
+    if (!h || !out3) return fail(DESIRE_ERR_ARG, "null argument");
+    for (int i = 0; i < 3; ++i) out3[i] = h->ioc_last[i];
+    return DESIRE_OK;
+}
+
 extern "C" int desire_set_profiling(desire_handle* h, int enable) {
     if (!h) return fail(DESIRE_ERR_ARG, "null handle");
     h->profiling = enable != 0;
diff --git a/desire_amd/csrc/api_forward.hip b/desire_amd/csrc/api_forward.hip
--- a/desire_amd/csrc/api_forward.hip
+++ b/desire_amd/csrc/api_forward.hip
@@ -395,6 +395,11 @@
         a.hex = W(h, "hex_s"); a.grp_cnt = Wt<int>(h, "cnt_s"); a.err = h->host_err;
         a.nspl = p.nspl;
     }
+    if (p.prepass) {
+        if (int rc = ws_ensure(h, {{"ioc_pre", ioc_pre_bytes((long)h->R, d.T_pred, d.E_v, d.C, d.grid_size * d.grid_size)}})) return rc;
+        a.pre = Wt<unsigned char>(h, "ioc_pre");
+    }
+    h->ioc_last[0] = (int)p.fwd; h->ioc_last[1] = p.nspl; h->ioc_last[2] = p.prepass ? 1 : 0;
 #ifdef DESIRE_IOC_TIMING
     if (int rc = ws_ensure(h, {{"dbg", 10 * sizeof(long long)}})) return rc;
     a.dbg = Wt<long long>(h, "dbg");
@@ -410,6 +415,7 @@
             if (p.cluster() && it > 0) { if (int rc = ioc_cluster_exchange(h, (size_t)v.R / v.mno, false, s)) return rc; }
         }
         Timer t(h, s, "ioc");
+        if (p.prepass) launch_ioc_pre(a, s);
         switch (p.fwd) {
             case IocFwd::FP32: case IocFwd::FP32_WIDE: launch_ioc(a, p.fwd == IocFwd::FP32_WIDE, s); break;
             case IocFwd::FP32_CLUSTER: launch_ioc_cluster(a, s); break;
diff --git a/desire_amd/csrc/ctx.h b/desire_amd/csrc/ctx.h
--- a/desire_amd/csrc/ctx.h
+++ b/desire_amd/csrc/ctx.h
@@ -54,6 +54,7 @@
     int* peer_err = nullptr;
     float head_loss_w = 0.f;
     int recon_mode = 0; float recon_tau = 0.f;
+    int ioc_last[3] = {-1, -1, -1};
     int* host_err = nullptr;
     int32_t* cp_host = nullptr; hipEvent_t cp_ev = nullptr; bool cp_pending = false; int cp_P = -1;
     int ci_cnt[4] = {0, 0, 0, 0}; bool ci_last = false; int ci_min_rows = 8192;
diff --git a/desire_amd/csrc/ioc_lds.h b/desire_amd/csrc/ioc_lds.h
--- a/desire_amd/csrc/ioc_lds.h
+++ b/desire_amd/csrc/ioc_lds.h
@@ -168,3 +168,12 @@
         return l;
     }
 };
+
+struct IocPreRec {
+    int nx, nmask, nrsrc;
+    IOC_HD constexpr int units() const { return nx + nmask + nrsrc + 1; }
+    IOC_HD constexpr size_t bytes() const { return (size_t)units() * 16; }
+};
+IOC_HD constexpr IocPreRec ioc_pre_rec(int EV, int C, int bins) { return IocPreRec{32 * (EV + C) / 4, 32 * bins / 4, (32 * bins + 15) / 16}; }
+IOC_HD constexpr size_t ioc_pre_bytes(long R, int T, int EV, int C, int bins) { return (size_t)((R + 31) / 32) * (size_t)T * ioc_pre_rec(EV, C, bins).bytes(); }
+IOC_HD constexpr int ioc_pre_sum_code(int slot) { return 32 + 1 + slot < 255 ? 32 + 1 + slot : 255; }
diff --git a/desire_amd/csrc/ioc_plan.h b/desire_amd/csrc/ioc_plan.h
--- a/desire_amd/csrc/ioc_plan.h
+++ b/desire_amd/csrc/ioc_plan.h
@@ -22,6 +22,11 @@
 }
 inline bool ioc_bwd_x3_supported(int mno, int H) { return mno <= 32 && (H == 64 || H == 128); }
 
+inline bool ioc_prepass_dims(const desire_dims& d) {
+    return d.bf16 == 0 && d.H <= 128 && d.mno <= 32 && d.iters == 1 && d.ioc_form == DESIRE_IOC_AUTO &&
+           !(d.flags & (DESIRE_FLAG_COMPACT_IOC | DESIRE_FLAG_IOC_NO_PREPASS));
+}
+
 enum class IocFwd { STEPWISE, FP32, FP32_WIDE, FP32_CLUSTER, BF16, BF16_WIDE, BF16_CLUSTER, X3, X3R2, X6, X6R2 };
 enum class IocBwd { FP32, X3, CLUSTER };
 
@@ -30,6 +35,7 @@
     int nspl = 1;
     IocBwd bwd = IocBwd::FP32;
     bool padded = false;
+    bool prepass = false;
     bool cluster() const { return fwd == IocFwd::FP32_CLUSTER || fwd == IocFwd::BF16_CLUSTER; }
     bool fp32_weights() const { return fwd == IocFwd::FP32 || fwd == IocFwd::FP32_WIDE || fwd == IocFwd::FP32_CLUSTER; }
 };
@@ -64,5 +70,6 @@
         while (n > 1 && (long)capacity(n) < tiles * n) --n;
         p.nspl = n;
     }
+    p.prepass = p.fwd == IocFwd::FP32 && !training && p.nspl == 1 && gpt == 0 && ioc_prepass_dims(d);
     return p;
 }
diff --git a/desire_amd/csrc/ioc_tile.h b/desire_amd/csrc/ioc_tile.h
--- a/desire_amd/csrc/ioc_tile.h
+++ b/desire_amd/csrc/ioc_tile.h
@@ -10,6 +10,10 @@
 
 #ifdef __HIPCC__
 #include "common.h"
+
+__device__ __forceinline__ float ioc_e_v(float vx, float vy, const float* wv, int j, int EV) {
+    return fmaxf(fmaf(vy, wv[EV + j], vx * wv[j]) + wv[2 * EV + j], 0.f);
+}
 
 #ifdef DESIRE_IOC_TIMING
 #define IOC_TICK(k) { const long long now_ = clock64(); tacc[k] += now_ - tprev; tprev = now_; }
diff --git a/desire_amd/csrc/kernels.h b/desire_amd/csrc/kernels.h
--- a/desire_amd/csrc/kernels.h
+++ b/desire_amd/csrc/kernels.h
@@ -139,8 +139,10 @@
     const float* bin_tab;
     int gpt; int ngrp;
     DynCount dyn;
+    unsigned char* pre;
 };
 void launch_ioc(const IocArgs& a, bool wide, hipStream_t s);
+void launch_ioc_pre(const IocArgs& a, hipStream_t s);
 void launch_ioc_cluster(const IocArgs& a, hipStream_t s);
 int ioc_bin_split_capacity(const IocArgs& a, int n);
 void launch_ioc_bf16(const IocArgs& a, bool wide, hipStream_t s);
diff --git a/desire_amd/csrc/kernels_ioc_pre.hip b/desire_amd/csrc/kernels_ioc_pre.hip
--- /dev/null
+++ b/desire_amd/csrc/kernels_ioc_pre.hip
@@ -0,0 +1,87 @@
+#include "kernels.h"
+#include "ioc_tile.h"
+
+constexpr int IOC_PRE_TS = 8;
+constexpr int IOC_PRE_MAX_BINS = 36;
+template <int EV, int C>
+__global__ __launch_bounds__(256) void k_ioc_pre(IocArgs a) {
+    constexpr int TM = 32, NTHR = 256, TPR = NTHR / TM;
+    constexpr IocPreRec LMAX = ioc_pre_rec(EV, C, IOC_PRE_MAX_BINS);
+    __shared__ uint4 meta[LMAX.nmask + LMAX.nrsrc + 1];
+    __shared__ float2 pos[(IOC_PRE_TS + 1) * TM];
+    __shared__ float wv[3 * EV];
+    __shared__ unsigned char vld[TM];
+    __shared__ int cnt[TM];
+    const int tid = threadIdx.x, r8 = tid / TPR, q8 = tid % TPR;
+    const int B = a.G * a.G;
+    const IocPreRec L = ioc_pre_rec(EV, C, B);
+    const int nmeta = L.nmask + L.nrsrc + 1;
+    unsigned* masks = reinterpret_cast<unsigned*>(meta);
+    unsigned char* rsrc = reinterpret_cast<unsigned char*>(meta + L.nmask);
+    unsigned* hdr = reinterpret_cast<unsigned*>(meta + L.nmask + L.nrsrc);
+    const int tile = blockIdx.x, row0 = tile * TM;
+    const int t0 = blockIdx.y * IOC_PRE_TS, t1 = min(t0 + IOC_PRE_TS, a.T);
+    const int my_row = min(row0 + r8, a.R - 1);
+    const int my_scene = my_row / (a.K * a.mno);
+    const int grp_base = (r8 / a.mno) * a.mno, my_slot = r8 - grp_base;
+
+    ioc_stage_wv<EV, NTHR>(wv, a.w_vel, a.b_vel, tid);
+    if (tid < TM) vld[tid] = a.valid[agent_of_row(min(row0 + tid, a.R - 1), a.K, a.mno)];
+    for (int i = tid; i < (t1 - t0 + 1) * TM; i += NTHR) {
+        const int s = i / TM, r = i - s * TM, t = t0 - 1 + s, row = min(row0 + r, a.R - 1);
+        pos[i] = t < 0 ? *reinterpret_cast<const float2*>(a.p_last + (size_t)agent_of_row(row, a.K, a.mno) * 2)
+                       : *reinterpret_cast<const float2*>(a.Y + ((size_t)row * a.T + t) * 2);
+    }
+    for (int i = tid; i < nmeta; i += NTHR) meta[i] = make_uint4(0u, 0u, 0u, 0u);
+    __syncthreads();
+    const float* grid = a.grids + (size_t)a.grid_of_scene[my_scene] * a.Gh * a.Gw * C;
+
+    for (int t = t0; t < t1; ++t) {
+        const float* pc = reinterpret_cast<const float*>(pos + (t - t0 + 1) * TM);
+        const float* pp = reinterpret_cast<const float*>(pos + (t - t0) * TM);
+        unsigned char* rec = a.pre + ((size_t)tile * a.T + t) * L.bytes();
+        {
+            float* x = reinterpret_cast<float*>(rec) + r8 * (EV + C);
+            const float px = pc[r8 * 2], py = pc[r8 * 2 + 1];
+            const float vx = px - pp[r8 * 2], vy = py - pp[r8 * 2 + 1];
+            constexpr int per = EV / TPR;
+            static_assert(per == 2 && C / TPR == 4, "a float2 of e_v and a float4 of e_s per thread");
+            *reinterpret_cast<float2*>(x + q8 * per) = make_float2(ioc_e_v(vx, vy, wv, q8 * per, EV), ioc_e_v(vx, vy, wv, q8 * per + 1, EV));
+            int cy, cx;
+            scene_cell_dev(px, py, a.Gh, a.Gw, cy, cx);
+            const float* gsrc = grid + ((size_t)cy * a.Gw + cx) * C;
+            *reinterpret_cast<float4*>(x + EV + q8 * 4) = *reinterpret_cast<const float4*>(gsrc + q8 * 4);
+            float nbw, nbh;
+            nb_opaque(a.nb_w, a.nb_h, nbw, nbh);
+            const unsigned long long oc = nb_search<4>(pc, vld, grp_base, a.mno, q8, TPR, my_slot, px, py, nbw, nbh, a.G, a.bin_tab,
+                                                      [&](int j, int b) { atomicOr(&masks[r8 * B + b], 1u << j); });
+            nb_publish_occ(oc, hdr, B);
+        }
+        __syncthreads();
+        unsigned mlo = 0u, mhi = 0u;
+        for (int b = q8; b < B; b += TPR) {
+            const int src = ioc_row_source(masks[r8 * B + b]);
+            if (src == IOC_ROW_SUM) { if (b < 32) mlo |= 1u << b; else mhi |= 1u << (b - 32); }
+            else rsrc[r8 * B + b] = (unsigned char)(src == IOC_ROW_ZERO ? TM : grp_base + src);
+        }
+#pragma unroll
+        for (int d = 1; d < TPR; d <<= 1) { mlo |= __shfl_xor(mlo, d); mhi |= __shfl_xor(mhi, d); }
+        const unsigned long long multi = ((unsigned long long)mhi << 32) | mlo;
+        if (q8 == 0) cnt[r8] = __popcll(multi);
+        __syncthreads();
+        int base = 0;
+        for (int i = 0; i < r8; ++i) base += cnt[i];
+        for (int b = q8; b < B; b += TPR)
+            if ((multi >> b) & 1ull) rsrc[r8 * B + b] = (unsigned char)ioc_pre_sum_code(base + __popcll(multi & ((1ull << b) - 1ull)));
+        if (tid == NTHR - 1) hdr[2] = (unsigned)(base + cnt[TM - 1]);
+        __syncthreads();
+        uint4* dst = reinterpret_cast<uint4*>(rec) + L.nx;
+        for (int i = tid; i < nmeta; i += NTHR) { dst[i] = meta[i]; meta[i] = make_uint4(0u, 0u, 0u, 0u); }
+        __syncthreads();
+    }
+}
+
+void launch_ioc_pre(const IocArgs& a, hipStream_t s) {
+    const dim3 grid((a.R + 31) / 32, (a.T + IOC_PRE_TS - 1) / IOC_PRE_TS);
+    hipLaunchKernelGGL((k_ioc_pre<16, 32>), grid, dim3(256), 0, s, a);
+}
diff --git a/desire_amd/csrc/kernels_rnn.hip b/desire_amd/csrc/kernels_rnn.hip
--- a/desire_amd/csrc/kernels_rnn.hip
+++ b/desire_amd/csrc/kernels_rnn.hip
@@ -384,7 +384,7 @@
         __builtin_amdgcn_sched_barrier(0);
     }
 }
-template <int H, int EV, int C, int TM, bool TRAIN, bool CP = false, int NSPL = 1, bool PAD = false>
+template <int H, int EV, int C, int TM, bool TRAIN, bool CP = false, int NSPL = 1, bool PAD = false, bool PRE = false>
 __global__ __launch_bounds__((H / 32) * (TM / 32) * 64, ((H / 32) * (TM / 32) <= 2) ? 1 : 2) void k_ioc(IocArgs a) {
 #ifdef DESIRE_IOC_TIMING
     long long tacc[10] = {0, 0, 0, 0, 0, 0, 0, 0, 0, 0};
@@ -414,6 +414,7 @@
     IOC_LDS_TIED(P0.off(P0.ROWLIST) - P0.off(P0.PC) == (TM * 2 * 2 + 3 * EV + NT * TM) * 4 + TM + (2 + 36) * 4);
     IOC_LDS_TIED(P0.sz[P0.ROWLIST] == 2 * (TM / 4) * 4);
     constexpr bool INPLACE = !CP && !(TM == 64 && ((H == 128 && TRAIN) || (H == 64 && !TRAIN)));
+    static_assert(!PRE || (INPLACE && TM == 32 && !TRAIN && NSPL == 1 && !PAD), "PRE: the dense 32-row inference form, rows read in place");
     constexpr int NSLOT = ioc_pool_slots(H, TM);
     unsigned char* rsrc = reinterpret_cast<unsigned char*>(AB + NSLOT * LDB);
     unsigned* nsum = rowbits;
@@ -439,9 +440,44 @@
     const int my_slot = r8 - grp_base;
     const int n_nb = dead_row ? 0 : a.mno;
 
-    ioc_stage_wv<EV, NTHR>(wv, a.w_vel, a.b_vel, tid);
+    if constexpr (!PRE) ioc_stage_wv<EV, NTHR>(wv, a.w_vel, a.b_vel, tid);
     for (int i = tid; i < LDX; i += NTHR) XH[TM * LDX + i] = 0.f;
-    if (tid < TM) { const int ag = ioc_agent_of_row(min(row0 + tid, a.R - 1), a.K, a.mno, gpt, a.ngrp); vld[tid] = ag >= 0 ? a.valid[ag] : 0; }
+    if (!PRE && tid < TM) { const int ag = ioc_agent_of_row(min(row0 + tid, a.R - 1), a.K, a.mno, gpt, a.ngrp); vld[tid] = ag >= 0 ? a.valid[ag] : 0; }
+    constexpr int NRX = (TM * (EV + C) / 4 + NTHR - 1) / NTHR, NRM = (ioc_pre_rec(EV, C, 36).units() - TM * (EV + C) / 4 + NTHR - 1) / NTHR;
+    const IocPreRec prl = ioc_pre_rec(EV, C, B);
+    static_assert(!PRE || P0.off(P0.ROWBITS) - P0.off(P0.OCC) == 8, "occ[2] and nsum are consecutive");
+    IOC_LDS_TIED(!PRE || (P0.off(P0.OCC) % 16 == 0 && (NSLOT * LDB * 4) % 16 == 0 && P0.off(P0.MASKS) % 16 == 0));
+    auto pre_rec = [&](int t) { return reinterpret_cast<const float4*>(a.pre + ((size_t)tile * a.T + t) * prl.bytes()); };
+    struct PreX { float4 v[NRX]; };
+    struct PreM { float4 v[NRM]; };
+    auto pre_load_x = [&](const float4* rec) {
+        PreX rx;
+#pragma unroll
+        for (int k = 0; k < NRX; ++k) rx.v[k] = rec[min(tid + k * NTHR, prl.nx - 1)];
+        return rx;
+    };
+    auto pre_load_m = [&](const float4* rec) {
+        PreM rm;
+#pragma unroll
+        for (int k = 0; k < NRM; ++k) rm.v[k] = rec[prl.nx + min(tid + k * NTHR, prl.units() - prl.nx - 1)];
+        return rm;
+    };
+    auto pre_store_x = [&](const PreX& rx) {
+#pragma unroll
+        for (int k = 0; k < NRX; ++k) {
+            const int i = tid + k * NTHR, r = i / ((EV + C) / 4), c4 = i - r * ((EV + C) / 4);
+            if (i < prl.nx) *reinterpret_cast<float4*>(XH + r * LDX + c4 * 4) = rx.v[k];
+        }
+    };
+    auto pre_store_m = [&](const PreM& rm) {
+#pragma unroll
+        for (int k = 0; k < NRM; ++k) {
+            const int i = tid + k * NTHR;
+            float4* dst = i < prl.nmask ? reinterpret_cast<float4*>(masks) + i
+                        : i < prl.nmask + prl.nrsrc ? reinterpret_cast<float4*>(rsrc) + (i - prl.nmask) : reinterpret_cast<float4*>(occ);
+            if (i < prl.units() - prl.nx) *dst = rm.v[k];
+        }
+    };
 
     float bgr = 0, bgu = 0, bcc = 0, bso = 0, wsc = 0;
     if (active) { bgr = a.b_g[col]; bgu = a.b_g[H + col]; bcc = a.b_c[col]; bso = a.b_soc[col]; wsc = a.w_score[col]; }
@@ -530,6 +566,44 @@
             if (q == 0) rsrc[r * B + b] = (unsigned char)(TM + 1 + slot);
         }
     };
+    auto pool_sums = [&]() {
+        int r = r8, q = q8, gb = grp_base;
+        asm volatile("" : "+v"(r), "+v"(q), "+v"(gb));
+        unsigned mlo = 0u, mhi = 0u;
+        for (int b = q; b < B; b += TPR)
+            if (rsrc[r * B + b] > TM) { if (b < 32) mlo |= 1u << b; else mhi |= 1u << (b - 32); }
+#pragma unroll
+        for (int d = 1; d < TPR; d <<= 1) { mlo |= __shfl_xor(mlo, d); if (B > 32) mhi |= __shfl_xor(mhi, d); }
+        unsigned long long multi = ((unsigned long long)mhi << 32) | mlo;
+        while (multi) {
+            const int b = ffs_(multi) - 1;
+            multi &= multi - 1;
+            const int slot = (int)rsrc[r * B + b] - (TM + 1);
+            mask_t m2 = masks[r * B + b];
+            const float* s0 = XH + (gb + ffs_(m2) - 1) * LDX + E + q * 4;
+            m2 &= m2 - 1;
+            const float* s1 = XH + (gb + ffs_(m2) - 1) * LDX + E + q * 4;
+            m2 &= m2 - 1;
+            float4 s[NCH];
+#pragma unroll
+            for (int c = 0; c < NCH; ++c) {
+                const float4 v0 = *reinterpret_cast<const float4*>(s0 + c * 4 * TPR);
+                const float4 v1 = *reinterpret_cast<const float4*>(s1 + c * 4 * TPR);
+                s[c].x = v0.x + v1.x; s[c].y = v0.y + v1.y; s[c].z = v0.z + v1.z; s[c].w = v0.w + v1.w;
+            }
+            while (m2) {
+                const float* src = XH + (gb + ffs_(m2) - 1) * LDX + E + q * 4;
+                m2 &= m2 - 1;
+#pragma unroll
+                for (int c = 0; c < NCH; ++c) {
+                    const float4 v = *reinterpret_cast<const float4*>(src + c * 4 * TPR);
+                    s[c].x += v.x; s[c].y += v.y; s[c].z += v.z; s[c].w += v.w;
+                }
+            }
+#pragma unroll
+            for (int c = 0; c < NCH; ++c) *reinterpret_cast<float4*>(AB + slot * LDB + q * 4 + c * 4 * TPR) = s[c];
+        }
+    };
 
     for (int it = 0; it < a.iters; ++it) {
         for (int i = tid; i < TM * (H >> 2); i += NTHR) {
@@ -538,7 +612,7 @@
             *reinterpret_cast<float4*>(XH + r * LDX + E + c4 * 4) =
                 ag >= 0 ? *reinterpret_cast<const float4*>(a.Hx + (size_t)ag * a.ldhx + c4 * 4) : make_float4(0.f, 0.f, 0.f, 0.f);
         }
-        if (tid < TM) {
+        if (!PRE && tid < TM) {
             const int ag = ioc_agent_of_row(min(row0 + tid, a.R - 1), a.K, a.mno, gpt, a.ngrp);
             pp[tid * 2] = ag >= 0 ? a.p_last[(size_t)ag * 2] : 0.f;
             pp[tid * 2 + 1] = ag >= 0 ? a.p_last[(size_t)ag * 2 + 1] : 0.f;
@@ -551,6 +625,11 @@
         }
 
         float2 ynext = make_float2(0.f, 0.f);
+        if constexpr (PRE) {
+            const PreX rx = pre_load_x(pre_rec(0));
+            const PreM rm = pre_load_m(pre_rec(0));
+            pre_store_x(rx); pre_store_m(rm);
+        } else {
         if (tid < TM) {
             const float2 y0 = *reinterpret_cast<const float2*>(a.Y + ((size_t)min(row0 + tid, a.R - 1) * a.T) * 2);
             pc[tid * 2] = y0.x; pc[tid * 2 + 1] = y0.y;
@@ -559,6 +638,7 @@
         if (tid < 2) occ[tid] = 0;
         if (INPLACE && tid == 2) *nsum = 0;
         if (CP && tid < B) rowbits[tid] = 0;
+        }
         __syncthreads();
         const float* rh_lane = AB + (mt * 32 + (lane & 31)) * LDB + 4 * (lane >> 5);
         float* my_rh = AB + (mt * 32 + 4 * (lane >> 5)) * LDB + col;
@@ -566,15 +646,15 @@
 
         for (int t = 0; t < a.T; ++t) {
             IOC_TICK(0)
-            if (tid < TM && t + 1 < a.T)
+            if (!PRE && tid < TM && t + 1 < a.T)
                 ynext = *reinterpret_cast<const float2*>(a.Y + ((size_t)min(row0 + tid, a.R - 1) * a.T + t + 1) * 2);
-            {
+            if constexpr (!PRE) {
                 const float px = pc[r8 * 2], py = pc[r8 * 2 + 1];
                 const float vx = px - pp[r8 * 2], vy = py - pp[r8 * 2 + 1];
                 constexpr int per = EV / TPR;
 #pragma unroll
                 for (int j = q8 * per; j < (q8 + 1) * per; ++j)
-                    XH[r8 * LDX + j] = fmaxf(fmaf(vy, wv[EV + j], vx * wv[j]) + wv[2 * EV + j], 0.f);
+                    XH[r8 * LDX + j] = ioc_e_v(vx, vy, wv, j, EV);
                 int cy, cx;
                 scene_cell_dev(px, py, a.Gh, a.Gw, cy, cx);
                 const float* gsrc = grid + ((size_t)cy * a.Gw + cx) * C;
@@ -600,7 +680,7 @@
                         *reinterpret_cast<float4*>(XH + r8 * LDX + EV + C + q8 * 4 + c * 4 * TPR) = make_float4(0.f, 0.f, 0.f, 0.f);
                 }
             }
-            __syncthreads();
+            if constexpr (!PRE) __syncthreads();
             IOC_TICK(1)
             if constexpr (CP) {
                 unsigned long long om = ioc_occ64(occ);
@@ -695,7 +775,12 @@
                 if (NSPL > 1) om &= my_bins;
                 int buf = 0;
                 bool in_place = false;
-                if constexpr (INPLACE) {
+                if constexpr (PRE) {
+                    const int ns = __builtin_amdgcn_readfirstlane((int)*nsum);
+                    if (ns > 0 && ns <= NSLOT) pool_sums();
+                    __syncthreads();
+                    in_place = ns <= NSLOT;
+                } else if constexpr (INPLACE) {
                     if (om) pool_rows(om);
                     __syncthreads();
                     in_place = __builtin_amdgcn_readfirstlane((int)*nsum) <= NSLOT;
@@ -808,6 +893,12 @@
             }
             __syncthreads();
             IOC_TICK(7)
+            PreX rx; PreM rm;
+            if constexpr (PRE) {
+                const float4* rec = pre_rec(min(t + 1, a.T - 1));
+                rm = pre_load_m(rec); rx = pre_load_x(rec);
+                __builtin_amdgcn_sched_barrier(0);
+            }
             if (active) {
                 f32x16 ac = zero16();
                 mma1(ac, x_lane, a.Wc + ((size_t)cb * G8) * 64 + lane, GX);
@@ -824,6 +915,11 @@
                     my_x[((i & 3) + 8 * (i >> 2)) * LDX + E] = h[i];
             }
             __builtin_amdgcn_s_setprio(0);
+            if constexpr (PRE) {
+                if (t + 1 < a.T) pre_store_m(rm);
+                __syncthreads();
+                if (t + 1 < a.T) pre_store_x(rx);
+            } else {
             if (tid < TM) {
                 pp[tid * 2] = pc[tid * 2]; pp[tid * 2 + 1] = pc[tid * 2 + 1];
                 pc[tid * 2] = ynext.x; pc[tid * 2 + 1] = ynext.y;
@@ -833,6 +929,7 @@
             if (INPLACE && tid == 2) *nsum = 0;
             if (CP && tid < B) rowbits[tid] = 0;
             __syncthreads();
+            }
             IOC_TICK(8)
         }
 #pragma unroll
@@ -914,6 +1011,10 @@
     if constexpr (TM == 32 && H <= 128) {
         if (a.gpt > 0) {
             launch_big_lds<k_ioc<H, 16, 32, 32, false, false, 1, true>>(grid, block, lds, s, a);
+            return;
+        }
+        if (a.pre) {
+            launch_big_lds<k_ioc<H, 16, 32, 32, false, false, 1, false, true>>(grid, block, lds, s, a);
             return;
         }
     }
diff --git a/desire_amd/spec.py b/desire_amd/spec.py
--- a/desire_amd/spec.py
+++ b/desire_amd/spec.py
@@ -14,6 +14,7 @@
 FLAG_COMPACT_ROWS = 4
 FLAG_COMPACT_IOC = 8
 FLAG_TRAIN_FWD_3P = 2
+FLAG_IOC_NO_PREPASS = 16
 
 
 @dataclass(frozen=True)
diff --git a/include/desire_hip.h b/include/desire_hip.h
--- a/include/desire_hip.h
+++ b/include/desire_hip.h
@@ -45,7 +45,11 @@
 
 #define DESIRE_FLAG_COMPACT_IOC 8
 
+#define DESIRE_FLAG_IOC_NO_PREPASS 16
+
 typedef struct desire_ctx desire_handle;
+
+int desire_ioc_plan_info(desire_handle* h, int32_t* out3);
 
 const char* desire_last_error(void);
 int desire_version(void);
```

After: 2.624 million samples/s. No clear change (-0.2%).
